# SDU-Gary/PCSS-Unet

Hardware: AMD Instinct MI355X
Metric: frames/sec 7x512x512 U-Net fwd+bwd (train step) (higher is better)
Workload: dtype f32; 1 GPU; configs[1]: batch=8/GPU 7x512x512 fp32 train step (fwd + 0.9*L1 + bwd + RCCL grad all-reduce + clip + AdamW); global_batch=8, in_ch=7, parallelism=dp1

## Files before the change

### include/nsm.h

```cpp
#ifndef NSM_H_
#define NSM_H_

#include <stddef.h>
#include <stdint.h>

#ifdef __cplusplus
extern "C" {
#endif

#define NSM_OK 0
#define NSM_E_ARG 1
#define NSM_E_HIP 2
#define NSM_E_WS 3

#define NSM_F32 0
#define NSM_BF16 1
#define NSM_F16 2

#define NSM_AMAX_WORDS 2048
#define NSM_PACK_FWD 0
#define NSM_PACK_DGRAD 1

int nsm_version(void);
int nsm_get_last_error(char* buf, size_t n);
// ... 84 lines not shown
                      const uint32_t* amax_dy, void* stream);
size_t nsm_wino_wgrad_f16_ws(int B, int H, int W, int cin_p, int cout_p, int tile);
int nsm_conv3x3_wgrad_wino_f16(const void* dM, const void* V, int B, int H, int W, int cin_p,
                               int cout_p, int cin, int cout, int tile, float* dw, float* ws,
                               size_t ws_floats, const uint32_t* amax_dy, const uint32_t* amax_x,
                               void* stream);
int nsm_wino_dual_input_bn_h2(const float* g, int ldg, const float* y, int ldy, int B, int H, int W,
                              int c_p, int tile, const float* scale, const float* shift,
                              float slope, const float* mask, const float* mean, const float* coef,
                              void* Vh, void* dMh, const uint32_t* bound, void* stream);
size_t nsm_wino_wgrad_h2_ws(int B, int H, int W, int cin_p, int cout_p, int tile);
int nsm_conv3x3_wgrad_wino_h2(const void* dMh, const void* Vh, int B, int H, int W, int cin_p,
                              int cout_p, int cin, int cout, int tile, float* dw, float* ws,
                              size_t ws_floats, const uint32_t* amax_dy, const uint32_t* amax_x,
                              void* stream);
int nsm_wino_gemm_h2(const void* V, const void* U, int B, int H, int W, int cin_p, int cout_p,
                     int tile, float* Mb, const uint32_t* amax_v, float beta_v,
                     const uint32_t* amax_u, float beta_u, void* stream);
int nsm_conv1x1_h2_rows(int M, int N, int K, int bnbwd);
int nsm_conv1x1_h2(const void* xh, int M, int cin_p, const void* wh, const float* bias, int cout_p,
                   float* y, int ldy, float* stats, const uint32_t* amax_x,
                   const uint32_t* amax_w, void* stream);
int nsm_conv1x1_dgrad_bnbwd_h2(const void* dy2h, int M, int cop, const void* w2dh, int cip,
                               const float* y1, int ldy1, const float* scale, const float* shift,
                               const float* mean, const float* invstd, const float* mask, int HW,
                               float slope, int mode, float* partial, const float* coef,
                               float* out, int ldo, const uint32_t* amax_dy2,
                               const uint32_t* amax_w, uint32_t* amax_out, uint32_t* amax_k1dz,
                               void* stream);
size_t nsm_conv1x1_wgrad_h2_ws(int M, int cin_p, int cout_p);
int nsm_conv1x1_wgrad_h2(const void* dyh, const void* xh, int M, int cin_p, int cout_p, int cin,
                         int cout, float* dw, float* ws, size_t ws_floats, const uint32_t* amax_dy,
                         const uint32_t* amax_x, void* stream);
int nsm_conv3x3_h2_rows(int M, int N);
int nsm_conv3x3_h2(const void* xh, int B, int H, int W, int cin_p, const void* wh,
                   const float* bias, int cout_p, float* y, int ldy, float* stats,
                   const uint32_t* amax_x, const uint32_t* amax_w, void* stream);
size_t nsm_conv3x3_wgrad_h2_ws(int B, int H, int W, int cin_p, int cout_p);
int nsm_conv3x3_wgrad_h2(const void* dyh, const void* xh, int B, int H, int W, int cin_p,
                         int cout_p, int cin, int cout, float* dw, float* ws, size_t ws_floats,
                         const uint32_t* amax_dy, const uint32_t* amax_x, void* stream);
int nsm_set_f32_split(int mode);
int nsm_wino_output(const float* Mb, int B, int H, int W, int cout_p, int tile, const float* bias,
                    float* y, int ldy, void* stream);
int nsm_wino_output_stats(const float* Mb, int B, int H, int W, int cout_p, int tile,
                          const float* bias, float* y, int ldy, float* partial, int nslot,
                          void* stream);
int nsm_wino_stat_slots(int B, int H, int W, int cout_p, int tile);
int nsm_wino_stat_step(int cout_p, int tile);

size_t nsm_wino_wgrad_ws(int B, int H, int W, int cin_p, int cout_p, int tile);
int nsm_conv3x3_wgrad_wino(const float* dy, int lddy, const float* V, int B, int H, int W,
                           int cin_p, int cout_p, int cin, int cout, int tile, float* dw,
                           float* ws, size_t ws_floats, void* stream);
int nsm_wino_dual_input(const float* dy, int lddy, int B, int H, int W, int c_p, int tile,
                        float* V, float* dM, uint32_t* amax_v, uint32_t* amax_dm, void* stream);
int nsm_wino_dual_input_bn(const float* g, int ldg, const float* y, int ldy, int B, int H, int W,
                           int c_p, int tile, const float* scale, const float* shift, float slope,
                           const float* mask, const float* mean, const float* coef, float* V,
                           float* dM, uint32_t* amax_v, uint32_t* amax_dm, void* stream);
int nsm_conv3x3_wgrad_wino_dm(const float* dM, const float* V, int B, int H, int W, int cin_p,
                              int cout_p, int cin, int cout, int tile, float* dw, float* ws,
                              size_t ws_floats, const uint32_t* amax_dm, const uint32_t* amax_v,
                              void* stream);

size_t nsm_conv_wgrad_ws(int B, int H, int W, int cin_p, int cout_p, int ksize);
int nsm_conv_wgrad(const float* dy, int lddy, const float* x, int ldx, int B, int H, int W,
                   int cin_p, int cout_p, int ksize, const float* pro_scale, const float* pro_shift,
                   const float* pro_mask, float slope, float* ws, size_t ws_floats, int cin, int cout,
                   float* dw, const uint32_t* amax_dy, const uint32_t* amax_x, void* stream);

int nsm_reduce_chunks(int M, int C);
int nsm_reduce_rows(int M, int C);
int nsm_bn_stats(const void* y, int ld, int M, int C, float* partial, int nchunk, int dtype,
                 void* stream);
int nsm_bn_finalize_train(const float* partial, int nchunk, int rows_per_chunk, int M, int C,
                          int c_real,
                          const float* gamma, const float* beta, float* run_mean, float* run_var,
                          int64_t* num_batches, float momentum, float eps, int n_updates,
                          float* mean, float* invstd, float* scale, float* shift, uint32_t* bound,
                          float bound_mul, void* stream);
int nsm_bn_partials_merge(const float* partial, int nchunk, int rows_per_chunk, int M, int C,
                          int group, float* out, void* stream);
int nsm_bn_finalize_eval(const float* run_mean, const float* run_var, const float* gamma,
                         const float* beta, int C, int c_real, float eps, float* mean,
                         float* invstd, float* scale, float* shift, void* stream);
int nsm_bn_act(const void* y, int ldy, int M, int C, const float* scale, const float* shift,
               float slope, const float* mask, int HW, const void* res, int ldres, void* out,
               int ldo, int dtype, uint32_t* amax, void* stream);
int nsm_bn_act_h2(const float* y, int ldy, int M, int C, const float* scale, const float* shift,
                  float slope, const float* mask, int HW, void* out, const uint32_t* bound,
                  void* stream);
int nsm_bn_bwd_reduce(const void* g, int ldg, const void* y, int ldy, int M, int C, int HW,
                      const float* scale, const float* shift, float slope, const float* mask,
                      const float* mean, const float* invstd, float* partial, int nchunk,
                      int dtype, uint32_t* amax_k1dz, void* stream);
int nsm_bn_bwd_finalize(const float* partial, int nchunk, int M, int C, int c_real,
                        const float* gamma, const float* invstd, float* dgamma, float* dbeta,
                        float* dbias_prev, float* coef, const uint32_t* amax_k1dz,
                        uint32_t* bound, void* stream);
int nsm_sum_rows(const float* part, int nrows, int width, int group, float* out, void* stream);
int nsm_bn_bwd_apply(const void* g, int ldg, const void* y, int ldy, int M, int C, int HW,
                     const float* scale, const float* shift, float slope, const float* mask,
                     const float* mean, const float* coef, void* dy, int lddy, int dtype,
                     uint32_t* amax, void* stream);
int nsm_bn_bwd_apply_h2(const float* g, int ldg, const float* y, int ldy, int M, int C, int HW,
                        const float* scale, const float* shift, float slope, const float* mask,
                        const float* mean, const float* coef, void* dy, const uint32_t* bound,
                        void* stream);

int nsm_avgpool2_fwd(const void* x, int B, int H, int W, int C, void* y, int dtype, void* stream);
int nsm_avgpool2_bwd_add(const void* dy, int B, int H, int W, int C, const void* skip, void* dx,
                         int dtype, void* stream);
int nsm_resize_fwd(const void* x, int B, int Hi, int Wi, int C, void* y, int Ho, int Wo, int dtype,
                   void* stream);
int nsm_resize_bwd(const void* dy, int B, int Hi, int Wi, int C, void* dx, int Ho, int Wo,
                   int dtype, void* stream);

int nsm_resize_fwd_act(const void* y2, int B, int Hi, int Wi, int C, void* out, int Ho, int Wo,
                       const float* scale, const float* shift, float slope, const void* res,
                       int dtype, void* stream);
int nsm_up2_resize_fwd_act(const void* y2, int B, int h, int w, int C, void* out, int th, int tw,
                           const float* scale, const float* shift, float slope, const void* res,
                           int dtype, void* stream);
int nsm_bn_act_pool(const void* y, int B, int H, int W, int C, const float* scale,
                    const float* shift, float slope, void* z, void* pooled, int dtype,
                    uint32_t* amax, void* stream);
int nsm_up2_resize_fwd(const void* x, int B, int h, int w, int C, void* y, int th, int tw,
                       int dtype, void* stream);
int nsm_up2_resize_bwd(const void* dy, int B, int h, int w, int C, void* dx, int th, int tw,
                       int dtype, void* stream);
int nsm_bnred_chunks(int kind, int B, int H, int W, int C);
int nsm_avgpool2_bwd_add_bnred(const void* dy, int B, int H, int W, int C, const void* skip,
                               void* dx, int dtype, const void* y2, const float* scale,
                               const float* shift, const float* mean, const float* invstd,
                               float slope, float* partial, uint32_t* amax_k1dz, void* stream);
int nsm_resize_bwd_bnred(const void* dy, int B, int Hi, int Wi, int C, void* dx, int Ho, int Wo,
                         int dtype, const void* y2, const float* scale, const float* shift,
                         const float* mean, const float* invstd, float slope, float* partial,
                         uint32_t* amax_k1dz, void* stream);
int nsm_up2_resize_bwd_bnred(const void* dy, int B, int h, int w, int C, void* dx, int th, int tw,
                             int dtype, const void* y2, const float* scale, const float* shift,
                             const float* mean, const float* invstd, float slope, float* partial,
                             uint32_t* amax_k1dz, void* stream);

int nsm_input_prep(const float* x, int B, int C, int H, int W, void* out, int cp, int dtype,
                   uint32_t* amax, void* stream);
int nsm_input_prep_h2(const float* x, int B, int C, int H, int W, void* out, int cp, uint32_t* amax,
                      void* stream);
int nsm_input_grad(const void* dX, int B, int C, int H, int W, int cp, float* dx, int dtype,
                   void* stream);
int nsm_head_fwd(const void* z, int ldz, int B, int Rh, int Rw, const float* w10,
                 const float* b10, float* out, int dtype, void* stream);
int nsm_head_bwd_blocks(int B, int Rh, int Rw);
int nsm_head_bwd(const float* gout, const float* out, const void* z, int ldz, int B, int Rh,
                 int Rw, const float* w10, void* dz, float* partial, float* dw10, float* db10,
                 int dtype, void* stream);

int nsm_loss_blocks(int64_t n);
int nsm_l1_loss_fwd(const float* o, const float* t, int64_t n, float alpha, float* partial,
                    float* out, void* stream);
int nsm_expdiff_mean(const float* a, const float* b, int64_t n, float alpha, float* partial,
                     float* out, void* stream);
int nsm_l1_loss_bwd(const float* o, const float* t, int64_t n, float alpha, const float* gscale,
                    float* grad, int accumulate, void* stream);
int nsm_detail_blocks(int B, int H, int W);
int nsm_detail_loss_fwd(const float* o, const float* t, int B, int H, int W, float w_hf,
                        float w_pen, float w_sob, const float* base, float* partial, float* out,
                        void* stream);
int nsm_detail_loss_bwd(const float* o, const float* t, int B, int H, int W, float w_hf,
                        float w_pen, float w_sob, const float* mcount, const float* gscale,
                        float* grad, int accumulate, void* stream);
int nsm_ssim_blocks(int B, int H, int W);
int nsm_ssim_fwd(const float* o, const float* t, int B, int H, int W, float data_range, float w,
                 const float* base, float* partial, float* coef, float* out, void* stream);
int nsm_ssim_bwd(const float* o, const float* t, const float* coef, int B, int H, int W, float w,
                 const float* gscale, float* grad, int accumulate, void* stream);
int nsm_temporal_blocks(int B, int C, int H, int W);
int nsm_temporal_pair(const float* cur, const float* prev, const float* mv, const float* depth_cur,
                      const float* depth_prev, const float* normal_cur, const float* normal_prev,
                      int B, int C, int H, int W, float scale_x, float scale_y, float alpha,
                      float depth_tol, float normal_cos, float* psum, int* pcnt, void* stream);
int nsm_temporal_finalize(const float* psum, const int* pcnt, int npairs, int B, int per,
                          int64_t all_count, float* sums, int64_t* counts, float* out, double* acc,
                          void* stream);
int nsm_reproject(const float* prev, const float* mv, int B, int C, int H, int W, float scale_x,
                  float scale_y, float* out, unsigned char* valid, void* stream);
int nsm_taa_resolve(const float* cur, const float* hist, const float* mv, const float* depth_cur,
                    const float* depth_prev, const float* normal_cur, const float* normal_prev,
                    int B, int C, int H, int W, float scale_x, float scale_y, float blend,
                    int clamp, float depth_tol, float normal_cos, float* out,
                    unsigned char* accepted, void* stream);
int nsm_sens_blocks(int64_t n);
int nsm_sens_variants(const float* x, const float* sigma, const int* channels,
                      const float* noises, uint64_t seed, int B, int C, int H, int W, int Cs,
                      int R, float factor, int first, int n, float* out, void* stream);
int nsm_sens_reduce(const float* out, const float* base, int first, int n_slots, int B, int Cs,
                    int R, int64_t n, float* psum, void* stream);
int nsm_sens_finalize(const float* psum, int Cs, int R, int B, int64_t n, const float* sigma,
                      const int* channels, float factor, float* terms, double* acc,
                      float* absolute, float* sgn, float* relative, void* stream);
int nsm_stats_blocks(int64_t hw);
int nsm_stats_partial(const float* x, int B, int C, int64_t HW, double* records, void* stream);
int nsm_stats_merge(const double* records, int B, int C, int per, double* frames, double* state,
                    void* stream);
#define NSM_METRICS_SCALARS 8
int nsm_metrics_blocks(int64_t n);
int nsm_metrics_partial(const float* o, const float* t, int B, int64_t n, float lo, float hi,
                        double* records, void* stream);
int nsm_metrics_merge(const double* records, int B, int per, const float* const* scalars, int K,
                      double* frames, double* log, int64_t log_capacity, double* state,
                      double* acc, void* stream);
int nsm_channel_std(const float* x, int B, int C, int H, int W, float* partial, float* std,
                    void* stream);
int nsm_perturb(const float* x, const float* noise, const float* std, int B, int C, int H,
                int W, float factor, float* out, void* stream);
#define NSM_PERT_MAX 8
int nsm_perturb_variants(const float* x, const float* std, const float* noises, uint64_t seed,
                         const int64_t* seed_dev, int P, int B, int C, int H, int W,
                         float factor, float* out, void* stream);
int nsm_pert_loss_blocks(int64_t n);
int nsm_pert_loss_fwd(const float* o, const float* t, const float* const* pouts, int P, int64_t n,
                      float alpha, float w, const float* vgg, float* partial, float* out,
                      void* stream);
int nsm_pert_loss_bwd(const float* o, const float* t, const float* const* pouts, int P, int64_t n,
                      float alpha, float w, const float* gscale, float* grad, int accumulate,
                      void* stream);

int nsm_sumsq(const float* g, int64_t n, float* partial, float* out, void* stream);
int nsm_clip_coef(const float* sumsq, float inv_world, float max_norm, float* coef, void* stream);
int nsm_adamw_step(float* p, const float* g, float* m, float* v, int64_t n, float lr, float beta1,
                   float beta2, float eps, float weight_decay, int step, const float* gcoef,
                   void* stream);
int nsm_adam_step(float* p, const float* g, float* m, float* v, int64_t n, float lr, float beta1,
                  float beta2, float eps, float weight_decay, int step, const float* gcoef,
                  void* stream);
int nsm_sgd_step(float* p, const float* g, float* buf, int64_t n, float lr, float momentum,
                 float weight_decay, int step, const float* gcoef, void* stream);

#define NSM_SCALER_WORDS 8
// ... 138 lines not shown
```

### pcss-unet_amd/csrc/nsm_elem.hip

```cpp
#include <algorithm>

#include "nsm_common.h"

namespace nsm {

static inline int gcd_i(int a, int b) {
  while (b) {
    int t = a % b;
    a = b;
    b = t;
  }
  return a;
}
struct ColRed {
  int cl, rl, gx, nchunk, rpc;
};
static ColRed colred_plan(int M, int C) {
  ColRed r;
  r.cl = gcd_i(C / 8, 64);
  r.rl = 256 / r.cl;
  r.gx = (C / 8) / r.cl;
  long long want = (M + 63) / 64;
  long long cap = 1024 / r.gx;
  if (cap < 1) cap = 1;
  r.nchunk = (int)(want < cap ? want : cap);
  if (r.nchunk < 1) r.nchunk = 1;
  r.rpc = ceil_div(M, r.nchunk);
  return r;
}

__device__ __forceinline__ void col_tree_reduce(F8* red, int cl, int rl, int tid) {
  for (int s = rl / 2; s > 0; s >>= 1) {
    __syncthreads();
    int tr = tid / cl;
    if (tr < s) red[tid] += red[tid + s * cl];
  }
  __syncthreads();
}

__device__ __forceinline__ F8 ldf8(const float* p) { return ld8(p); }

template <typename T>
__global__ void __launch_bounds__(256) bn_stats_kernel(const T* __restrict__ y, int ld, int M,
                                                       int C, int cl, int rl, int rpc,
                                                       float* __restrict__ partial) {
  __shared__ F8 red[256];
  const int tid = threadIdx.x, tc = tid % cl, tr = tid / cl;
  const int c = (blockIdx.x * cl + tc) * 8;
  const int r0 = blockIdx.y * rpc, r1 = min(M, r0 + rpc);
  F8 s = f8zero();
#pragma unroll 4
  for (int r = r0 + tr; r < r1; r += rl) s += ld8(y + (size_t)r * ld + c);
  red[tid] = s;
  col_tree_reduce(red, cl, rl, tid);
  const float n = (float)max(r1 - r0, 1);
  const F8 sum = red[tc];
  const F8 mean = (1.f / n) * sum;
  __syncthreads();
  F8 s2 = f8zero();
#pragma unroll 4
  for (int r = r0 + tr; r < r1; r += rl) {
    F8 d = ld8(y + (size_t)r * ld + c) - mean;
    s2 += d * d;
  }
  red[tid] = s2;
  col_tree_reduce(red, cl, rl, tid);
  if (tr == 0) {
    float* pr = partial + (size_t)blockIdx.y * 2 * C;
    st8(pr + c, sum);
    st8(pr + C + c, red[tc]);
  }
}

__device__ __forceinline__ double wave_sum_d(double v) {
#pragma unroll
  for (int o = 32; o > 0; o >>= 1) v += __shfl_xor(v, o, 64);
  return v;
}

__device__ __forceinline__ double block_sum_d(double v, double* red) {
  v = wave_sum_d(v);
  __syncthreads();
  if ((threadIdx.x & 63) == 0) red[threadIdx.x >> 6] = v;
  __syncthreads();
  return (red[0] + red[1]) + (red[2] + red[3]);
}

__global__ void __launch_bounds__(256) bn_finalize_train_kernel(
    const float* __restrict__ partial, int nchunk, int rpc, int M, int C, int c_real,
    const float* __restrict__ gamma, const float* __restrict__ beta, float* run_mean,
    float* run_var, int64_t* num_batches, float momentum, float eps, int n_updates, float* mean_o,
    float* invstd_o, float* scale_o, float* shift_o, uint32_t* bound, float bound_mul) {
  __shared__ double red[4];
  const int tid = threadIdx.x;
  const int c = blockIdx.x;
  if (blockIdx.x == 0 && tid == 0 && num_batches) *num_batches += n_updates;
  const size_t st = (size_t)(rpc ? 2 : 3) * C;
  double s0 = 0.0, s1 = 0.0, s2 = 0.0, s3 = 0.0;
  int k = tid;
  for (; k + 768 < nchunk; k += 1024) {
    s0 += partial[k * st + c];
    s1 += partial[(k + 256) * st + c];
    s2 += partial[(k + 512) * st + c];
    s3 += partial[(k + 768) * st + c];
  }
  for (; k < nchunk; k += 256) s0 += partial[k * st + c];
  const double mean = block_sum_d((s0 + s1) + (s2 + s3), red) / M;
  double q0 = 0.0, q1 = 0.0;
  for (k = tid; k < nchunk; k += 512) {
    int n0 = rpc ? min(M, k * rpc + rpc) - k * rpc : (int)partial[k * st + 2 * C + c];
    if (n0 > 0) {
      double d = partial[k * st + c] / n0 - mean;
      q0 += partial[k * st + C + c] + n0 * d * d;
    }
    int k1 = k + 256;
    if (k1 < nchunk) {
      int n1 = rpc ? min(M, k1 * rpc + rpc) - k1 * rpc : (int)partial[k1 * st + 2 * C + c];
      if (n1 > 0) {
        double d = partial[k1 * st + c] / n1 - mean;
        q1 += partial[k1 * st + C + c] + n1 * d * d;
      }
    }
  }
  const double m2 = block_sum_d(q0 + q1, red);
  if (tid != 0) return;
  const float var_b = (float)(m2 / M);
  const float var_u = M > 1 ? (float)(m2 / (M - 1)) : var_b;
  const float mf = (float)mean;
  const float inv = 1.0f / sqrtf(var_b + eps);
  const float sc = gamma[c] * inv;
  mean_o[c] = mf;
  invstd_o[c] = inv;
  scale_o[c] = sc;
  shift_o[c] = beta[c] - mf * sc;
  if (bound) {
    const double b = ((double)fabsf(sc) * sqrt((double)var_b * (double)(M - 1)) +
                      (double)fabsf(beta[c])) * (double)bound_mul * (1.0 + 1e-6);
    atomicMax(bound + (c & (AMAX_LINES - 1)) * AMAX_STRIDE, __float_as_uint((float)b) & 0x7fffffffu);
  }
  if (c < c_real && run_mean) {
    float rm = run_mean[c], rv = run_var[c];
    for (int u = 0; u < n_updates; ++u) {
      rm = momentum * mf + (1.f - momentum) * rm;
      rv = momentum * var_u + (1.f - momentum) * rv;
    }
    run_mean[c] = rm;
    run_var[c] = rv;
  }
}

__global__ void bn_partials_merge_kernel(const float* __restrict__ partial, int nchunk, int rpc,
                                         int M, int C, int G, float* __restrict__ out) {
  const int c = blockIdx.x * blockDim.x + threadIdx.x;
  const int g = blockIdx.y;
  if (c >= C) return;
  const size_t st = (size_t)(rpc ? 2 : 3) * C;
  const int k0 = g * G, k1 = min(nchunk, k0 + G);
  double s = 0.0;
  long long n = 0;
  for (int k = k0; k < k1; ++k) {
    s += partial[(size_t)k * st + c];
    n += rpc ? max(0, min(M, (k + 1) * rpc) - k * rpc) : (long long)partial[(size_t)k * st + 2 * C + c];
  }
  const double mean = n > 0 ? s / (double)n : 0.0;
  double m2 = 0.0;
  for (int k = k0; k < k1; ++k) {
    const int nk = rpc ? min(M, (k + 1) * rpc) - k * rpc : (int)partial[(size_t)k * st + 2 * C + c];
    if (nk <= 0) continue;
    const double d = partial[(size_t)k * st + c] / nk - mean;
    m2 += partial[(size_t)k * st + C + c] + nk * d * d;
  }
  out[(size_t)g * st + c] = (float)s;
  out[(size_t)g * st + C + c] = (float)m2;
  if (!rpc) out[(size_t)g * st + 2 * C + c] = (float)n;
}

__global__ void sum_rows_kernel(const float* __restrict__ part, int nrows, int width, int G,
                                float* __restrict__ out) {
  const int j = blockIdx.x * blockDim.x + threadIdx.x, g = blockIdx.y;
  if (j >= width) return;
  const int k0 = g * G, k1 = min(nrows, k0 + G);
  double s = 0.0, s1 = 0.0;
  int k = k0;
  for (; k + 1 < k1; k += 2) {
    s += part[(size_t)k * width + j];
    s1 += part[(size_t)(k + 1) * width + j];
  }
  if (k < k1) s += part[(size_t)k * width + j];
  out[(size_t)g * width + j] = (float)(s + s1);
}

__global__ void bn_finalize_eval_kernel(const float* __restrict__ rm, const float* __restrict__ rv,
                                        const float* __restrict__ gamma,
                                        const float* __restrict__ beta, int C, int c_real, float eps,
                                        float* mean_o, float* invstd_o, float* scale_o,
                                        float* shift_o) {
  int c = blockIdx.x * blockDim.x + threadIdx.x;
  if (c >= C) return;
  float m = c < c_real ? rm[c] : 0.f;
  float v = c < c_real ? rv[c] : 1.f;
  float inv = 1.0f / sqrtf(v + eps);
  float sc = gamma[c] * inv;
  mean_o[c] = m;
  invstd_o[c] = inv;
  scale_o[c] = sc;
  shift_o[c] = beta[c] - m * sc;
}

__device__ __forceinline__ f32x4 lrelu4(f32x4 v, float slope) {
  return f32x4{lrelu(v.x, slope), lrelu(v.y, slope), lrelu(v.z, slope), lrelu(v.w, slope)};
}
__device__ __forceinline__ F8 lrelu8(F8 v, float slope) {
  return F8{lrelu4(v.a, slope), lrelu4(v.b, slope)};
}

template <typename T>
__global__ void __launch_bounds__(256) bn_act_kernel(const T* __restrict__ y, int ldy, int M,
                                                     int C8, FastDiv fdHW,
                                                     const float* __restrict__ scale,
                                                     const float* __restrict__ shift, float slope,
                                                     const float* __restrict__ mask,
                                                     const T* __restrict__ res, int ldres,
                                                     T* __restrict__ out, int ldo,
                                                     uint32_t* __restrict__ amax) {
  const int ppb = blockDim.x / C8, tp = threadIdx.x / C8;
  const int c = (threadIdx.x - tp * C8) * 8;
  const F8 sc = ldf8(scale + c), sh = ldf8(shift + c);
  const int pstep = gridDim.x * ppb;
  uint32_t am = 0;
  for (int p = blockIdx.x * ppb + tp; p < M; p += pstep) {
    F8 o = lrelu8(ld8(y + (size_t)p * ldy + c) * sc + sh, slope);
    if (mask) o = o * ld8(mask + (size_t)fdiv((uint32_t)p, fdHW) * (C8 * 8) + c);
    if (res) o += ld8(res + (size_t)p * ldres + c);
    st8(out + (size_t)p * ldo + c, o);
    if (amax) {
      amax_fold(am, o.a);
      amax_fold(am, o.b);
    }
  }
  amax_flush(am, amax);
}

__global__ void __launch_bounds__(256) bn_act_h2_kernel(const float* __restrict__ y, int ldy, int M,
                                                        int C8, FastDiv fdHW,
                                                        const float* __restrict__ scale,
                                                        const float* __restrict__ shift,
                                                        float slope,
                                                        const float* __restrict__ mask,
                                                        bf16_t* __restrict__ out, H2Scale hs) {
  const float s = exp2i(h2_exp(hs));
  const int ppb = blockDim.x / C8, tp = threadIdx.x / C8;
  const int c = (threadIdx.x - tp * C8) * 8;
  const F8 sc = ldf8(scale + c), sh = ldf8(shift + c);
  const int pstep = gridDim.x * ppb;
  for (int p = blockIdx.x * ppb + tp; p < M; p += pstep) {
    F8 o = lrelu8(ld8(y + (size_t)p * ldy + c) * sc + sh, slope);
    if (mask) o = o * ld8(mask + (size_t)fdiv((uint32_t)p, fdHW) * (C8 * 8) + c);
    h2_store8(out + (size_t)p * 16 * C8, c, o, s);
  }
}

__device__ __forceinline__ f32x4 lrelu_grad4(f32x4 z, float slope) {
  return f32x4{lrelu_grad(z.x, slope), lrelu_grad(z.y, slope), lrelu_grad(z.z, slope),
               lrelu_grad(z.w, slope)};
}
__device__ __forceinline__ F8 bn_dz8(const F8 g, const F8 v, const F8 sc, const F8 sh,
                                     float slope, const float* mask, int b, int C, int c) {
  const F8 z = v * sc + sh;
  F8 d{g.a * lrelu_grad4(z.a, slope), g.b * lrelu_grad4(z.b, slope)};
  if (mask) d = d * ld8(mask + (size_t)b * C + c);
  return d;
}

template <typename T>
__global__ void __launch_bounds__(256) bn_bwd_reduce_kernel(
    const T* __restrict__ g, int ldg, const T* __restrict__ y, int ldy, int M, int C,
    FastDiv fdHW, const float* __restrict__ scale, const float* __restrict__ shift, float slope,
    const float* __restrict__ mask, const float* __restrict__ mean,
    const float* __restrict__ invstd, int cl, int rl, int rpc, float* __restrict__ partial,
    uint32_t* __restrict__ amax) {
  __shared__ F8 red[256];
  const int tid = threadIdx.x, tc = tid % cl, tr = tid / cl;
  const int c = (blockIdx.x * cl + tc) * 8;
  const int r0 = blockIdx.y * rpc, r1 = min(M, r0 + rpc);
  const F8 sc = ldf8(scale + c), sh = ldf8(shift + c);
  const F8 mu = ldf8(mean + c), is = ldf8(invstd + c);
  F8 s1 = f8zero(), s2 = f8zero();
  uint32_t am = 0;
#pragma unroll 2
  for (int r = r0 + tr; r < r1; r += rl) {
    const F8 v = ld8(y + (size_t)r * ldy + c);
    const F8 gg = ld8(g + (size_t)r * ldg + c);
    const int b = mask ? (int)fdiv((uint32_t)r, fdHW) : 0;
    const F8 dz = bn_dz8(gg, v, sc, sh, slope, mask, b, C, c);
    s1 += dz;
    s2 += dz * ((v - mu) * is);
    if (amax) {
      amax_fold(am, sc.a * dz.a);
      amax_fold(am, sc.b * dz.b);
    }
  }
  amax_flush(am, amax);
  red[tid] = s1;
  col_tree_reduce(red, cl, rl, tid);
  const F8 t1 = red[tc];
  __syncthreads();
  red[tid] = s2;
  col_tree_reduce(red, cl, rl, tid);
  if (tr == 0) {
    float* pr = partial + (size_t)blockIdx.y * 2 * C;
    st8(pr + c, t1);
    st8(pr + C + c, red[tc]);
  }
}

__global__ void __launch_bounds__(256) bn_bwd_finalize_kernel(
    const float* __restrict__ partial, int nchunk, int M, int C, int c_real,
    const float* __restrict__ gamma, const float* __restrict__ invstd, float* dgamma,
    float* dbeta, float* dbias_prev, float* coef, const uint32_t* __restrict__ amax_k1dz,
    uint32_t* __restrict__ bound) {
  __shared__ double red[4];
  const int tid = threadIdx.x;
  const int c = blockIdx.x;
  const float a_k1dz = bound ? __uint_as_float(amax_read(amax_k1dz)) : 0.f;
  const size_t st = (size_t)2 * C;
  double a0 = 0.0, a1 = 0.0, b0 = 0.0, b1 = 0.0;
  int k = tid;
  for (; k + 256 < nchunk; k += 512) {
    a0 += partial[k * st + c];
    b0 += partial[k * st + C + c];
    a1 += partial[(k + 256) * st + c];
    b1 += partial[(k + 256) * st + C + c];
  }
  for (; k < nchunk; k += 256) {
    a0 += partial[k * st + c];
    b0 += partial[k * st + C + c];
  }
  const double S1 = block_sum_d(a0 + a1, red), S2 = block_sum_d(b0 + b1, red);
  if (tid != 0) return;
  const float gm = gamma[c], is = invstd[c];
  const double mdz = S1 / M, mdzx = S2 / M;
  const float k1 = gm * is;
  const float k2 = (float)(-(double)gm * is * is * mdzx);
  const float k3 = (float)(-(double)k1 * mdz);
  coef[c] = k1;
  coef[C + c] = k2;
  coef[2 * C + c] = k3;
  if (bound) {
    const double b = ((double)a_k1dz + fabs((double)k2) * sqrt((double)(M - 1)) / (double)is +
                      fabs((double)k3)) * (1.0 + 1e-6);
    atomicMax(bound + (c & (AMAX_LINES - 1)) * AMAX_STRIDE, __float_as_uint((float)b) & 0x7fffffffu);
  }
  if (c < c_real) {
    if (dgamma) dgamma[c] = (float)S2;
    if (dbeta) dbeta[c] = (float)S1;
    if (dbias_prev) dbias_prev[c] = (float)((double)k1 * S1 + (double)k3 * M);
  }
}

template <typename T>
__global__ void __launch_bounds__(256) bn_bwd_apply_kernel(
    const T* __restrict__ g, int ldg, const T* __restrict__ y, int ldy, int M, int C, int C8,
    FastDiv fdHW, const float* __restrict__ scale, const float* __restrict__ shift, float slope,
    const float* __restrict__ mask, const float* __restrict__ mean,
    const float* __restrict__ coef, T* __restrict__ dy, int lddy, uint32_t* __restrict__ amax) {
  const int ppb = blockDim.x / C8, tp = threadIdx.x / C8;
  const int c = (threadIdx.x - tp * C8) * 8;
  const F8 sc = ldf8(scale + c), sh = ldf8(shift + c), mu = ldf8(mean + c);
  const F8 k1 = ldf8(coef + c), k2 = ldf8(coef + C + c), k3 = ldf8(coef + 2 * C + c);
  const int pstep = gridDim.x * ppb;
  uint32_t am = 0;
  for (int p = blockIdx.x * ppb + tp; p < M; p += pstep) {
    const F8 v = ld8(y + (size_t)p * ldy + c);
    const F8 gg = ld8(g + (size_t)p * ldg + c);
    const int b = mask ? (int)fdiv((uint32_t)p, fdHW) : 0;
    const F8 dz = bn_dz8(gg, v, sc, sh, slope, mask, b, C, c);
    const F8 d = k1 * dz + k2 * (v - mu) + k3;
    st8(dy + (size_t)p * lddy + c, d);
    if (amax) {
      amax_fold(am, d.a);
      amax_fold(am, d.b);
    }
  }
  amax_flush(am, amax);
}

__global__ void __launch_bounds__(256) bn_bwd_apply_h2_kernel(
    const float* __restrict__ g, int ldg, const float* __restrict__ y, int ldy, int M, int C,
    int C8, FastDiv fdHW, const float* __restrict__ scale, const float* __restrict__ shift,
    float slope, const float* __restrict__ mask, const float* __restrict__ mean,
    const float* __restrict__ coef, bf16_t* __restrict__ dy, H2Scale hs) {
  const float s = exp2i(h2_exp(hs));
  const int ppb = blockDim.x / C8, tp = threadIdx.x / C8;
  const int c = (threadIdx.x - tp * C8) * 8;
  const F8 sc = ldf8(scale + c), sh = ldf8(shift + c), mu = ldf8(mean + c);
  const F8 k1 = ldf8(coef + c), k2 = ldf8(coef + C + c), k3 = ldf8(coef + 2 * C + c);
  const int pstep = gridDim.x * ppb;
  for (int p = blockIdx.x * ppb + tp; p < M; p += pstep) {
    const F8 v = ld8(y + (size_t)p * ldy + c);
    const F8 gg = ld8(g + (size_t)p * ldg + c);
    const int b = mask ? (int)fdiv((uint32_t)p, fdHW) : 0;
    const F8 dz = bn_dz8(gg, v, sc, sh, slope, mask, b, C, c);
    h2_store8(dy + (size_t)p * 2 * C, c, k1 * dz + k2 * (v - mu) + k3, s);
  }
}

struct BnRedP {
  const void* y;
  const float* scale;
  const float* shift;
  const float* mean;
  const float* invstd;
  float slope;
  float* partial;
  uint32_t* amax;
};
template <typename T>
__device__ __forceinline__ F8 as_stored8(F8 v);
template <>
__device__ __forceinline__ F8 as_stored8<float>(F8 v) { return v; }
template <>
__device__ __forceinline__ F8 as_stored8<f16_t>(F8 v) {
  const u32x4 w = u32x4{pack_hh(v.a.x, v.a.y), pack_hh(v.a.z, v.a.w), pack_hh(v.b.x, v.b.y),
                        pack_hh(v.b.z, v.b.w)};
  return F8{f32x4{h_lo(w.x), h_hi(w.x), h_lo(w.y), h_hi(w.y)},
            f32x4{h_lo(w.z), h_hi(w.z), h_lo(w.w), h_hi(w.w)}};
}
template <>
__device__ __forceinline__ F8 as_stored8<bf16_t>(F8 v) {
  const u32x4 w = u32x4{pack_bf2(v.a.x, v.a.y), pack_bf2(v.a.z, v.a.w), pack_bf2(v.b.x, v.b.y),
                        pack_bf2(v.b.z, v.b.w)};
  return F8{f32x4{bf_lo(w.x), bf_hi(w.x), bf_lo(w.y), bf_hi(w.y)},
            f32x4{bf_lo(w.z), bf_hi(w.z), bf_lo(w.w), bf_hi(w.w)}};
}
struct BnRedAcc {
  F8 sc, sh, mu, is, s1, s2;
  uint32_t am;
  __device__ void init(const BnRedP& r, int c) {
    sc = ldf8(r.scale + c);
    sh = ldf8(r.shift + c);
    mu = ldf8(r.mean + c);
    is = ldf8(r.invstd + c);
    s1 = f8zero();
    s2 = f8zero();
    am = 0;
  }
  template <typename T>
  __device__ void add(const BnRedP& r, F8 g, size_t p, int C, int c) {
    const F8 v = ld8((const T*)r.y + p * C + c);
    const F8 dz = bn_dz8(g, v, sc, sh, r.slope, nullptr, 0, C, c);
    s1 += dz;
    s2 += dz * ((v - mu) * is);
    if (r.amax) {
      amax_fold(am, sc.a * dz.a);
      amax_fold(am, sc.b * dz.b);
    }
  }
  __device__ void write(const BnRedP& r, int C8) {
    __shared__ F8 red[256];
    const int tid = threadIdx.x, rl = 256 / C8, tc = tid % C8, C = C8 * 8;
    red[tid] = s1;
    col_tree_reduce(red, C8, rl, tid);
    const F8 t1 = red[tc];
    __syncthreads();
    red[tid] = s2;
    col_tree_reduce(red, C8, rl, tid);
    if (tid < C8) {
      float* pr = r.partial + (size_t)blockIdx.x * 2 * C;
      st8(pr + tc * 8, t1);
      st8(pr + C + tc * 8, red[tc]);
    }
    amax_flush(am, r.amax);
  }
  __device__ void write_slice(const BnRedP& r, int G, int c0, int C, int row) {
    __shared__ F8 red[256];
    const int tid = threadIdx.x, rl = 256 / G, tc = tid % G;
    red[tid] = s1;
    col_tree_reduce(red, G, rl, tid);
    const F8 t1 = red[tc];
    __syncthreads();
    red[tid] = s2;
    col_tree_reduce(red, G, rl, tid);
    if (tid < G) {
      float* pr = r.partial + (size_t)row * 2 * C + c0;
      st8(pr + tc * 8, t1);
      st8(pr + C + tc * 8, red[tc]);
    }
    amax_flush(am, r.amax);
  }
};

template <typename T>
__global__ void __launch_bounds__(256) avgpool2_fwd_kernel(const T* __restrict__ x, int B, int H,
                                                           int W, int C8, FastDiv fdC8,
                                                           FastDiv fdWo, FastDiv fdHo,
                                                           T* __restrict__ y) {
  const int Ho = H / 2, Wo = W / 2, C = C8 * 8;
  const uint32_t total = (uint32_t)B * Ho * Wo * C8;
  for (uint32_t i = blockIdx.x * 256u + threadIdx.x; i < total; i += gridDim.x * 256u) {
    const uint32_t p = fdiv(i, fdC8);
    const int c = (int)(i - p * (uint32_t)C8) * 8;
    const uint32_t t = fdiv(p, fdWo);
    const int ox = (int)(p - t * Wo);
    const uint32_t b = fdiv(t, fdHo);
    const int oy = (int)(t - b * Ho);
    const T* base = x + (((size_t)b * H + 2 * oy) * W + 2 * ox) * C + c;
    const size_t rs = (size_t)W * C;
    F8 s = ld8(base);
    s += ld8(base + C);
    s += ld8(base + rs);
    s += ld8(base + rs + C);
    st8(y + (size_t)p * C + c, 0.25f * s);
  }
}

template <typename T>
__global__ void __launch_bounds__(256) bn_act_pool_kernel(const T* __restrict__ y, int B, int H,
                                                          int W, int C8, FastDiv fdC8,
                                                          FastDiv fdWc, FastDiv fdHc,
                                                          const float* __restrict__ scale,
                                                          const float* __restrict__ shift,
                                                          float slope, T* __restrict__ z,
                                                          T* __restrict__ pooled,
                                                          uint32_t* __restrict__ amax) {
  const int Hc = (H + 1) / 2, Wc = (W + 1) / 2, Ho = H / 2, Wo = W / 2, C = C8 * 8;
  uint32_t am = 0;
  const uint32_t total = (uint32_t)B * Hc * Wc * C8;
  for (uint32_t i = blockIdx.x * 256u + threadIdx.x; i < total; i += gridDim.x * 256u) {
    const uint32_t p = fdiv(i, fdC8);
    const int c = (int)(i - p * (uint32_t)C8) * 8;
    const uint32_t t = fdiv(p, fdWc);
    const int cx = (int)(p - t * Wc);
// ... 783 lines not shown
template <bool COMP>
static void dispatch_sep_bwd(const SepPlan& pl, int B, size_t lds, hipStream_t s, const void* dy,
                             int h, int w, int C, void* dx, int th, int tw, float s1h, float s1w,
                             float s2h, float s2w, const BnRedP* rp, int dtype) {
  const dim3 g((unsigned)(B * ((h + pl.R - 1) / pl.R)), (unsigned)(C >> (pl.lcb8 + 3)));
  const BnRedP r = rp ? *rp : BnRedP{};
#define NSM_SEP(T, RED, R)                                                                      \
  launch_sep_bwd<T, RED, COMP, R>(g, lds, s, dy, h, w, C, pl.lcb8, dx, th, tw, s1h, s1w, s2h, s2w, r)
#define NSM_SEP_R(T, RED) \
  (pl.R == 4 ? NSM_SEP(T, RED, 4) : pl.R == 2 ? NSM_SEP(T, RED, 2) : NSM_SEP(T, RED, 1))
  if (dtype == NSM_BF16) {
    if (rp) NSM_SEP_R(bf16_t, true); else NSM_SEP_R(bf16_t, false);
  }
  else if (dtype == NSM_F16) {
    if (rp) NSM_SEP_R(f16_t, true); else NSM_SEP_R(f16_t, false);
  } else {
    if (rp) NSM_SEP_R(float, true); else NSM_SEP_R(float, false);
  }
#undef NSM_SEP_R
#undef NSM_SEP
}
static int sep_resize_mode() { static const int v = (int)env_int("NSM_RESIZE_SEP", 1); return v; }
static bool sep_resize() { return sep_resize_mode() != 0; }
static bool sep_for(int dtype) { return dtype == NSM_F32 ? sep_resize() : sep_resize_mode() == 2; }

template <typename T, bool H2 = false>
__global__ void __launch_bounds__(256) input_prep_kernel(const float* __restrict__ x, int B, int C,
                                                         int H, int W, T* __restrict__ out, int cp,
                                                         uint32_t npix, FastDiv fdRw, FastDiv fdRh,
                                                         uint32_t* __restrict__ amax) {
  const int Rh = H / 2, Rw = W / 2;
  const size_t plane = (size_t)H * W;
  float hs = 0.f;
  if constexpr (H2) hs = exp2i(h2_exp(H2Scale{amax, 1.f}));
  uint32_t am = 0;
  for (uint32_t p = blockIdx.x * 256u + threadIdx.x; p < npix; p += gridDim.x * 256u) {
    const uint32_t t = fdiv(p, fdRw);
    const int rx = (int)(p - t * (uint32_t)Rw);
    const uint32_t b = fdiv(t, fdRh);
    const int ry = (int)(t - b * (uint32_t)Rh);
    const float* src = x + (size_t)b * C * plane + (size_t)(2 * ry) * W + 2 * rx;
    for (int g = 0; g < cp / 8; ++g) {
      f32x2 r[4];
#pragma unroll
      for (int q = 0; q < 4; ++q) {
        const int c = 2 * g + (q >> 1);
        r[q] = c < C ? *(const f32x2*)(src + (size_t)c * plane + (q & 1) * W) : f32x2{0.f, 0.f};
      }
      const F8 v{f32x4{r[0].x, r[0].y, r[1].x, r[1].y}, f32x4{r[2].x, r[2].y, r[3].x, r[3].y}};
      if constexpr (H2) {
        h2_store8((bf16_t*)out + (size_t)p * 2 * cp, 8 * g, v, hs);
      } else {
        st8(out + (size_t)p * cp + 8 * g, v);
        if (amax) {
          amax_fold(am, v.a);
          amax_fold(am, v.b);
        }
      }
    }
  }
  if constexpr (!H2) amax_flush(am, amax);
}

template <typename T>
__global__ void input_grad_kernel(const T* __restrict__ dX, int B, int C, int H, int W, int cp,
                                  float* __restrict__ dx) {
  const int Rh = H / 2, Rw = W / 2;
  long long total = (long long)B * C * Rh * Rw;
  long long i = (long long)blockIdx.x * blockDim.x + threadIdx.x;
  for (; i < total; i += (long long)gridDim.x * blockDim.x) {
    int rx = (int)(i % Rw);
    long long t = i / Rw;
    int ry = (int)(t % Rh);
    t /= Rh;
    int c = (int)(t % C);
    int b = (int)(t / C);
    f32x4 v = ld4(dX + (((size_t)b * Rh + ry) * Rw + rx) * cp + 4 * c);
    float* o = dx + (((size_t)b * C + c) * H + 2 * ry) * W + 2 * rx;
    *(f32x2*)o = f32x2{v.x, v.y};
    *(f32x2*)(o + W) = f32x2{v.z, v.w};
  }
}

template <typename T>
__global__ void head_fwd_kernel(const T* __restrict__ z, int ldz, int B, int Rh, int Rw,
                                const float* __restrict__ w10, const float* __restrict__ b10,
                                float* __restrict__ out) {
  __shared__ float w[68];
  if (threadIdx.x < 64) w[threadIdx.x] = w10[threadIdx.x];
  if (threadIdx.x < 4) w[64 + threadIdx.x] = b10[threadIdx.x];
  __syncthreads();
  long long npix = (long long)B * Rh * Rw;
  for (long long p = (long long)blockIdx.x * blockDim.x + threadIdx.x; p < npix;
       p += (long long)gridDim.x * blockDim.x) {
    float zz[16];
    const T* zr = z + (size_t)p * ldz;
#pragma unroll
    for (int q = 0; q < 4; ++q) {
      f32x4 v = ld4(zr + 4 * q);
      zz[4 * q] = v.x;
      zz[4 * q + 1] = v.y;
      zz[4 * q + 2] = v.z;
      zz[4 * q + 3] = v.w;
    }
    int rx = (int)(p % Rw);
    long long t = p / Rw;
    int ry = (int)(t % Rh);
    int b = (int)(t / Rh);
#pragma unroll
    for (int j = 0; j < 4; ++j) {
      float acc = 0.f;
#pragma unroll
      for (int c = 0; c < 16; ++c) acc += w[j * 16 + c] * zz[c];
      acc += w[64 + j];
      float s = 1.f / (1.f + expf(-acc));
      int di = j >> 1, dj = j & 1;
      out[((size_t)b * 2 * Rh + 2 * ry + di) * (2 * Rw) + 2 * rx + dj] = s;
    }
  }
}

__device__ __forceinline__ float wave_sum(float v) {
#pragma unroll
  for (int o = 32; o > 0; o >>= 1) v += __shfl_xor(v, o, 64);
  return v;
}

template <typename T>
__global__ void __launch_bounds__(256) head_bwd_kernel(
    const float* __restrict__ gout, const float* __restrict__ out, const T* __restrict__ z,
    int ldz, int B, int Rh, int Rw, const float* __restrict__ w10, T* __restrict__ dz,
    float* __restrict__ partial) {
  __shared__ float w[64];
  __shared__ float red[4][68];
  if (threadIdx.x < 64) w[threadIdx.x] = w10[threadIdx.x];
  __syncthreads();
  float accw[68];
#pragma unroll
  for (int k = 0; k < 68; ++k) accw[k] = 0.f;
  long long npix = (long long)B * Rh * Rw;
  for (long long p = (long long)blockIdx.x * blockDim.x + threadIdx.x; p < npix;
       p += (long long)gridDim.x * blockDim.x) {
    int rx = (int)(p % Rw);
    long long t = p / Rw;
    int ry = (int)(t % Rh);
    int b = (int)(t / Rh);
    float d[4];
#pragma unroll
    for (int di = 0; di < 2; ++di) {
      size_t o = ((size_t)b * 2 * Rh + 2 * ry + di) * (2 * Rw) + 2 * rx;
      const f32x2 ov = *(const f32x2*)(out + o), gv = *(const f32x2*)(gout + o);
      d[2 * di] = gv.x * (1.f - ov.x) * ov.x;
      d[2 * di + 1] = gv.y * (1.f - ov.y) * ov.y;
    }
    const T* zr = z + (size_t)p * ldz;
    T* dzr = dz + (size_t)p * ldz;
#pragma unroll
    for (int q = 0; q < 4; ++q) {
      f32x4 v = ld4(zr + 4 * q);
      float zv[4] = {v.x, v.y, v.z, v.w};
      f32x4 g;
      float gv[4];
#pragma unroll
      for (int e = 0; e < 4; ++e) {
        int c = 4 * q + e;
        gv[e] = d[0] * w[c] + d[1] * w[16 + c] + d[2] * w[32 + c] + d[3] * w[48 + c];
#pragma unroll
        for (int j = 0; j < 4; ++j) accw[j * 16 + c] += d[j] * zv[e];
      }
      g.x = gv[0];
      g.y = gv[1];
      g.z = gv[2];
      g.w = gv[3];
      st4(dzr + 4 * q, g);
    }
    for (int c = 16; c < ldz; c += 4) st4(dzr + c, f32x4{0.f, 0.f, 0.f, 0.f});
#pragma unroll
    for (int j = 0; j < 4; ++j) accw[64 + j] += d[j];
  }
  const int lane = threadIdx.x & 63, wv = threadIdx.x >> 6;
#pragma unroll
  for (int o = 32; o >= 1; o >>= 1) {
    const bool up = (lane & o) != 0;
#pragma unroll
    for (int i = 0; i < o; ++i) {
      const float lo = accw[i], hi = accw[i + o];
      accw[i] = (up ? hi : lo) + __shfl_xor(up ? lo : hi, o, 64);
    }
  }
  red[wv][lane] = accw[0];
#pragma unroll
  for (int k = 64; k < 68; ++k) {
    float s = wave_sum(accw[k]);
    if (lane == 0) red[wv][k] = s;
  }
  __syncthreads();
  if (threadIdx.x < 68) {
    float s = red[0][threadIdx.x] + red[1][threadIdx.x] + red[2][threadIdx.x] + red[3][threadIdx.x];
    partial[(size_t)blockIdx.x * 68 + threadIdx.x] = s;
  }
}

__global__ void __launch_bounds__(256) head_reduce_kernel(const float* __restrict__ partial,
                                                          int nblk, float* dw10, float* db10) {
  __shared__ double sh[256];
  const int j = blockIdx.x;
  double s = 0.0;
  for (int b = threadIdx.x; b < nblk; b += 256) s += partial[(size_t)b * 68 + j];
  sh[threadIdx.x] = s;
  __syncthreads();
  for (int o = 128; o > 0; o >>= 1) {
    if ((int)threadIdx.x < o) sh[threadIdx.x] += sh[threadIdx.x + o];
    __syncthreads();
  }
  if (threadIdx.x == 0) {
    if (j < 64)
      dw10[j] = (float)sh[0];
    else
      db10[j - 64] = (float)sh[0];
  }
}

__device__ __forceinline__ float block_sum256(float v, float* sh) {
  v = wave_sum(v);
  const int lane = threadIdx.x & 63, wv = threadIdx.x >> 6;
  __syncthreads();
  if (lane == 0) sh[wv] = v;
  __syncthreads();
  float r = 0.f;
  if (threadIdx.x == 0) {
    for (int k = 0; k < (int)(blockDim.x >> 6); ++k) r += sh[k];
  }
  return r;
}

__global__ void __launch_bounds__(256) l1_partial_kernel(const float* __restrict__ o,
                                                         const float* __restrict__ t, int64_t n,
                                                         float* __restrict__ partial) {
  __shared__ float sh[4];
  float s = 0.f;
  for (int64_t i = (int64_t)blockIdx.x * blockDim.x + threadIdx.x; i < n;
       i += (int64_t)gridDim.x * blockDim.x)
    s += fabsf(o[i] - t[i]);
  float r = block_sum256(s, sh);
  if (threadIdx.x == 0) partial[blockIdx.x] = r;
}

__global__ void __launch_bounds__(256) expdiff_partial_kernel(const float* __restrict__ a,
                                                              const float* __restrict__ b,
                                                              int64_t n, float alpha,
                                                              float* __restrict__ partial) {
  __shared__ float sh[4];
  float s = 0.f;
  for (int64_t i = (int64_t)blockIdx.x * blockDim.x + threadIdx.x; i < n;
       i += (int64_t)gridDim.x * blockDim.x)
    s += expf(alpha * fabsf(a[i] - b[i])) - 1.f;
  float r = block_sum256(s, sh);
  if (threadIdx.x == 0) partial[blockIdx.x] = r;
}

__global__ void finalize_mean_kernel(const float* __restrict__ partial, int nblk, double scale,
                                     float* out) {
  __shared__ double sh[64];
  double s = 0.0;
  for (int b = threadIdx.x; b < nblk; b += 64) s += partial[b];
  sh[threadIdx.x] = s;
  __syncthreads();
  if (threadIdx.x == 0) {
    double tot = 0.0;
    for (int k = 0; k < 64; ++k) tot += sh[k];
    out[0] = (float)(tot * scale);
  }
}

__global__ void l1_bwd_kernel(const float* __restrict__ o, const float* __restrict__ t, int64_t n,
                              float alpha, const float* __restrict__ gscale, float* grad,
                              int accumulate) {
  const float gs = gscale ? gscale[0] : 1.f;
  const float mag = (alpha * gs) / (float)n;
  for (int64_t i = (int64_t)blockIdx.x * blockDim.x + threadIdx.x; i < n;
       i += (int64_t)gridDim.x * blockDim.x) {
    float d = o[i] - t[i];
// ... 125 lines not shown
                           float* __restrict__ buf, int64_t n, float lr, float momentum, float wd,
                           int first, const float* __restrict__ gcoef) {
#pragma clang fp contract(off)
  const float gc = gcoef ? gcoef[0] : 1.f;
  for (int64_t i = (int64_t)blockIdx.x * blockDim.x + threadIdx.x; i < n;
       i += (int64_t)gridDim.x * blockDim.x) {
    float pi = p[i];
    float gi = g[i] * gc;
    gi = gi + wd * pi;
    if (MOMENTUM) {
      if (!first) gi = buf[i] * momentum + gi;
      buf[i] = gi;
    }
    p[i] = pi - lr * gi;
  }
}

static inline int xcd_grid(long long work) {
  long long g = (work + 255) / 256;
  g = g > 2048 ? 2048 : g;
  return (int)((g + 7) / 8 * 8);
}

static inline int grid_for(long long work, int per_block = 256, int cap = 8192) {
  long long g = (work + per_block - 1) / per_block;
  if (g < 1) g = 1;
  if (g > cap) g = cap;
  return (int)g;
}

}

using namespace nsm;

extern "C" int nsm_reduce_chunks(int M, int C) {
  if (M <= 0 || C <= 0 || C % 8) return 0;
  return colred_plan(M, C).nchunk;
}

#define NSM_T(T, p) ((T*)(p))
#define NSM_CT(T, p) ((const T*)(p))

extern "C" int nsm_bn_stats(const void* y, int ld, int M, int C, float* partial, int nchunk,
                            int dtype, void* stream) {
  NSM_CHECK_ARG(y && partial && M > 0 && C % 8 == 0 && ld % 8 == 0, "bn_stats: bad args");
  ColRed r = colred_plan(M, C);
  NSM_CHECK_ARG(nchunk == r.nchunk, "bn_stats: nchunk %d != %d", nchunk, r.nchunk);
  dim3 g(r.gx, r.nchunk);
  if (dtype == NSM_BF16)
    hipLaunchKernelGGL(bn_stats_kernel<bf16_t>, g, dim3(256), 0, as_stream(stream),
                       NSM_CT(bf16_t, y), ld, M, C, r.cl, r.rl, r.rpc, partial);
  else if (dtype == NSM_F16)
    hipLaunchKernelGGL(bn_stats_kernel<f16_t>, g, dim3(256), 0, as_stream(stream),
                       NSM_CT(f16_t, y), ld, M, C, r.cl, r.rl, r.rpc, partial);
  else
    hipLaunchKernelGGL(bn_stats_kernel<float>, g, dim3(256), 0, as_stream(stream),
                       NSM_CT(float, y), ld, M, C, r.cl, r.rl, r.rpc, partial);
  NSM_LAUNCH_CHECK("bn_stats");
  return 0;
}

extern "C" int nsm_reduce_rows(int M, int C) {
  if (M <= 0 || C <= 0 || C % 8) return 0;
  return colred_plan(M, C).rpc;
}

extern "C" int nsm_bn_finalize_train(const float* partial, int nchunk, int rows_per_chunk, int M,
                                     int C, int c_real, const float* gamma, const float* beta,
                                     float* run_mean, float* run_var, int64_t* num_batches,
                                     float momentum, float eps, int n_updates, float* mean,
                                     float* invstd, float* scale, float* shift, uint32_t* bound,
                                     float bound_mul, void* stream) {
  NSM_CHECK_ARG(partial && gamma && beta && mean && invstd && scale && shift, "bn_finalize: null");
  NSM_CHECK_ARG(M > 1, "bn_finalize: Expected more than 1 value per channel when training");
  NSM_CHECK_ARG(nchunk >= 1 && (rows_per_chunk == 0 ||
                                (rows_per_chunk >= 1 && (long long)nchunk * rows_per_chunk >= M)),
                "bn_finalize: chunks do not cover M");
  hipLaunchKernelGGL(bn_finalize_train_kernel, dim3(C), dim3(256), 0,
                     as_stream(stream), partial, nchunk, rows_per_chunk, M, C, c_real, gamma, beta,
                     run_mean,
                     run_var, num_batches, momentum, eps, n_updates, mean, invstd, scale, shift,
                     bound, bound_mul);
  NSM_LAUNCH_CHECK("bn_finalize_train");
  return 0;
}

extern "C" int nsm_bn_partials_merge(const float* partial, int nchunk, int rows_per_chunk, int M,
                                     int C, int group, float* out, void* stream) {
  NSM_CHECK_ARG(partial && out && nchunk >= 1 && group >= 1 && rows_per_chunk >= 0,
                "bn_partials_merge: bad args");
  dim3 grid(ceil_div(C, 256), ceil_div(nchunk, group));
  hipLaunchKernelGGL(bn_partials_merge_kernel, grid, dim3(256), 0, as_stream(stream), partial,
                     nchunk, rows_per_chunk, M, C, group, out);
  NSM_LAUNCH_CHECK("bn_partials_merge");
  return 0;
}

extern "C" int nsm_sum_rows(const float* part, int nrows, int width, int group, float* out,
                            void* stream) {
  NSM_CHECK_ARG(part && out && nrows >= 1 && width >= 1 && group >= 1, "sum_rows: bad args");
  dim3 grid(ceil_div(width, 256), ceil_div(nrows, group));
  hipLaunchKernelGGL(sum_rows_kernel, grid, dim3(256), 0, as_stream(stream), part, nrows, width,
                     group, out);
  NSM_LAUNCH_CHECK("sum_rows");
  return 0;
}

extern "C" int nsm_bn_finalize_eval(const float* run_mean, const float* run_var,
                                    const float* gamma, const float* beta, int C, int c_real,
                                    float eps, float* mean, float* invstd, float* scale,
                                    float* shift, void* stream) {
  NSM_CHECK_ARG(run_mean && run_var && gamma && beta && scale && shift, "bn_finalize_eval: null");
  hipLaunchKernelGGL(bn_finalize_eval_kernel, dim3(ceil_div(C, 256)), dim3(256), 0,
                     as_stream(stream), run_mean, run_var, gamma, beta, C, c_real, eps, mean, invstd,
                     scale, shift);
  NSM_LAUNCH_CHECK("bn_finalize_eval");
  return 0;
}

static void pix_launch(long long M, int C8, dim3& grid, dim3& block) {
  const int tpb = (256 / C8) * C8;
  const long long ppb = tpb / C8;
  long long g = (M + ppb - 1) / ppb;
  g = g < 1 ? 1 : (g > 2048 ? 2048 : g);
  grid = dim3((unsigned)g);
  block = dim3((unsigned)tpb);
}

extern "C" int nsm_bn_act(const void* y, int ldy, int M, int C, const float* scale,
                          const float* shift, float slope, const float* mask, int HW,
                          const void* res, int ldres, void* out, int ldo, int dtype,
                          uint32_t* amax, void* stream) {
  NSM_CHECK_ARG(y && scale && shift && out && C % 8 == 0 && C <= 2048 && ldy % 8 == 0 &&
                    ldo % 8 == 0 && (!res || ldres % 8 == 0) && (!mask || HW > 0),
                "bn_act: bad args");
  NSM_CHECK_ARG(M >= 0 && M < (1 << 30), "bn_act: too large");
  if (M == 0) return 0;
  dim3 g, b;
  pix_launch(M, C / 8, g, b);
  const FastDiv fh = make_fastdiv(mask ? HW : 1);
  if (dtype == NSM_BF16)
    hipLaunchKernelGGL(bn_act_kernel<bf16_t>, g, b, 0, as_stream(stream), NSM_CT(bf16_t, y), ldy,
                       M, C / 8, fh, scale, shift, slope, mask, NSM_CT(bf16_t, res), ldres,
                       NSM_T(bf16_t, out), ldo, amax);
  else if (dtype == NSM_F16)
    hipLaunchKernelGGL(bn_act_kernel<f16_t>, g, b, 0, as_stream(stream), NSM_CT(f16_t, y), ldy,
                       M, C / 8, fh, scale, shift, slope, mask, NSM_CT(f16_t, res), ldres,
                       NSM_T(f16_t, out), ldo, amax);
  else
    hipLaunchKernelGGL(bn_act_kernel<float>, g, b, 0, as_stream(stream), NSM_CT(float, y), ldy, M,
                       C / 8, fh, scale, shift, slope, mask, NSM_CT(float, res), ldres,
                       NSM_T(float, out), ldo, amax);
  NSM_LAUNCH_CHECK("bn_act");
  return 0;
}

extern "C" int nsm_bn_act_h2(const float* y, int ldy, int M, int C, const float* scale,
                             const float* shift, float slope, const float* mask, int HW, void* out,
                             const uint32_t* bound, void* stream) {
  NSM_CHECK_ARG(y && scale && shift && out && bound && C % 8 == 0 && C <= 2048 && ldy % 8 == 0 &&
                    (!mask || HW > 0) && ((uintptr_t)out % 16) == 0,
                "bn_act_h2: bad args");
  NSM_CHECK_ARG(M >= 0 && M < (1 << 30), "bn_act_h2: too large");
  if (M == 0) return 0;
  dim3 g, b;
  pix_launch(M, C / 8, g, b);
  hipLaunchKernelGGL(bn_act_h2_kernel, g, b, 0, as_stream(stream), y, ldy, M, C / 8,
                     make_fastdiv(mask ? HW : 1), scale, shift, slope, mask, (bf16_t*)out,
                     H2Scale{bound, 1.f});
  NSM_LAUNCH_CHECK("bn_act_h2");
  return 0;
}

extern "C" int nsm_bn_bwd_reduce(const void* g, int ldg, const void* y, int ldy, int M, int C,
                                 int HW, const float* scale, const float* shift, float slope,
                                 const float* mask, const float* mean, const float* invstd,
                                 float* partial, int nchunk, int dtype, uint32_t* amax_k1dz,
                                 void* stream) {
  NSM_CHECK_ARG(g && y && scale && shift && mean && invstd && partial && C % 8 == 0 &&
                    ldg % 8 == 0 && ldy % 8 == 0, "bn_bwd_reduce: bad args");
  ColRed r = colred_plan(M, C);
  NSM_CHECK_ARG(nchunk == r.nchunk, "bn_bwd_reduce: nchunk mismatch");
  dim3 gr(r.gx, r.nchunk);
  if (dtype == NSM_BF16)
    hipLaunchKernelGGL(bn_bwd_reduce_kernel<bf16_t>, gr, dim3(256), 0, as_stream(stream),
                       NSM_CT(bf16_t, g), ldg, NSM_CT(bf16_t, y), ldy, M, C, make_fastdiv(HW),
                       scale, shift, slope, mask, mean, invstd, r.cl, r.rl, r.rpc, partial,
                       amax_k1dz);
  else if (dtype == NSM_F16)
    hipLaunchKernelGGL(bn_bwd_reduce_kernel<f16_t>, gr, dim3(256), 0, as_stream(stream),
                       NSM_CT(f16_t, g), ldg, NSM_CT(f16_t, y), ldy, M, C, make_fastdiv(HW),
                       scale, shift, slope, mask, mean, invstd, r.cl, r.rl, r.rpc, partial,
                       amax_k1dz);
  else
    hipLaunchKernelGGL(bn_bwd_reduce_kernel<float>, gr, dim3(256), 0, as_stream(stream),
                       NSM_CT(float, g), ldg, NSM_CT(float, y), ldy, M, C, make_fastdiv(HW), scale,
                       shift, slope, mask, mean, invstd, r.cl, r.rl, r.rpc, partial, amax_k1dz);
  NSM_LAUNCH_CHECK("bn_bwd_reduce");
  return 0;
}

extern "C" int nsm_bn_bwd_finalize(const float* partial, int nchunk, int M, int C, int c_real,
                                   const float* gamma, const float* invstd, float* dgamma,
                                   float* dbeta, float* dbias_prev, float* coef,
                                   const uint32_t* amax_k1dz, uint32_t* bound, void* stream) {
  NSM_CHECK_ARG(partial && gamma && invstd && coef, "bn_bwd_finalize: bad args");
  NSM_CHECK_ARG(!bound || amax_k1dz, "bn_bwd_finalize: a bound needs the max|k1 dz| slot");
  NSM_CHECK_ARG(M > 1 || !bound, "bn_bwd_finalize: M");
  hipLaunchKernelGGL(bn_bwd_finalize_kernel, dim3(C), dim3(256), 0,
                     as_stream(stream), partial, nchunk, M, C, c_real, gamma, invstd, dgamma, dbeta,
                     dbias_prev, coef, amax_k1dz, bound);
  NSM_LAUNCH_CHECK("bn_bwd_finalize");
  return 0;
}

extern "C" int nsm_bn_bwd_apply(const void* g, int ldg, const void* y, int ldy, int M, int C,
                                int HW, const float* scale, const float* shift, float slope,
                                const float* mask, const float* mean, const float* coef, void* dy,
                                int lddy, int dtype, uint32_t* amax, void* stream) {
  NSM_CHECK_ARG(g && y && scale && shift && mean && coef && dy && C % 8 == 0 && C <= 2048 &&
                    ldg % 8 == 0 && ldy % 8 == 0 && lddy % 8 == 0 && (!mask || HW > 0),
                "bn_bwd_apply: bad args");
  NSM_CHECK_ARG(M >= 0 && M < (1 << 30), "bn_bwd_apply: too large");
  if (M == 0) return 0;
  dim3 gr, b;
  pix_launch(M, C / 8, gr, b);
  const FastDiv fh = make_fastdiv(mask ? HW : 1);
  if (dtype == NSM_BF16)
    hipLaunchKernelGGL(bn_bwd_apply_kernel<bf16_t>, gr, b, 0, as_stream(stream),
                       NSM_CT(bf16_t, g), ldg, NSM_CT(bf16_t, y), ldy, M, C, C / 8, fh, scale,
                       shift, slope, mask, mean, coef, NSM_T(bf16_t, dy), lddy, amax);
  else if (dtype == NSM_F16)
    hipLaunchKernelGGL(bn_bwd_apply_kernel<f16_t>, gr, b, 0, as_stream(stream),
                       NSM_CT(f16_t, g), ldg, NSM_CT(f16_t, y), ldy, M, C, C / 8, fh, scale,
                       shift, slope, mask, mean, coef, NSM_T(f16_t, dy), lddy, amax);
  else
    hipLaunchKernelGGL(bn_bwd_apply_kernel<float>, gr, b, 0, as_stream(stream),
                       NSM_CT(float, g), ldg, NSM_CT(float, y), ldy, M, C, C / 8, fh, scale,
                       shift, slope, mask, mean, coef, NSM_T(float, dy), lddy, amax);
  NSM_LAUNCH_CHECK("bn_bwd_apply");
  return 0;
}

extern "C" int nsm_bn_bwd_apply_h2(const float* g, int ldg, const float* y, int ldy, int M, int C,
                                   int HW, const float* scale, const float* shift, float slope,
                                   const float* mask, const float* mean, const float* coef,
                                   void* dy, const uint32_t* bound, void* stream) {
  NSM_CHECK_ARG(g && y && scale && shift && mean && coef && dy && bound && C % 8 == 0 &&
                    C <= 2048 && ldg % 8 == 0 && ldy % 8 == 0 && (!mask || HW > 0) &&
                    ((uintptr_t)dy % 16) == 0,
                "bn_bwd_apply_h2: bad args");
  NSM_CHECK_ARG(M >= 0 && M < (1 << 30), "bn_bwd_apply_h2: too large");
  if (M == 0) return 0;
  dim3 gr, b;
  pix_launch(M, C / 8, gr, b);
  hipLaunchKernelGGL(bn_bwd_apply_h2_kernel, gr, b, 0, as_stream(stream), g, ldg, y, ldy, M, C,
                     C / 8, make_fastdiv(mask ? HW : 1), scale, shift, slope, mask, mean, coef,
                     (bf16_t*)dy, H2Scale{bound, 1.f});
  NSM_LAUNCH_CHECK("bn_bwd_apply_h2");
  return 0;
}

extern "C" int nsm_bn_act_pool(const void* y, int B, int H, int W, int C, const float* scale,
                               const float* shift, float slope, void* z, void* pooled, int dtype,
                               uint32_t* amax, void* stream) {
  NSM_CHECK_ARG(y && z && pooled && scale && shift && C % 8 == 0 && H >= 2 && W >= 2,
                "bn_act_pool: bad args");
  const long long work = (long long)B * ((H + 1) / 2) * ((W + 1) / 2) * (C / 8);
  NSM_CHECK_ARG(work < (1ll << 31), "bn_act_pool: too large");
  dim3 g(grid_for(work));
  const FastDiv f8 = make_fastdiv(C / 8), fw = make_fastdiv((W + 1) / 2),
                fh = make_fastdiv((H + 1) / 2);
  if (dtype == NSM_BF16)
    hipLaunchKernelGGL(bn_act_pool_kernel<bf16_t>, g, dim3(256), 0, as_stream(stream),
                       NSM_CT(bf16_t, y), B, H, W, C / 8, f8, fw, fh, scale, shift, slope,
                       NSM_T(bf16_t, z), NSM_T(bf16_t, pooled), amax);
  else if (dtype == NSM_F16)
    hipLaunchKernelGGL(bn_act_pool_kernel<f16_t>, g, dim3(256), 0, as_stream(stream),
                       NSM_CT(f16_t, y), B, H, W, C / 8, f8, fw, fh, scale, shift, slope,
                       NSM_T(f16_t, z), NSM_T(f16_t, pooled), amax);
  else
    hipLaunchKernelGGL(bn_act_pool_kernel<float>, g, dim3(256), 0, as_stream(stream),
                       NSM_CT(float, y), B, H, W, C / 8, f8, fw, fh, scale, shift, slope,
                       NSM_T(float, z), NSM_T(float, pooled), amax);
  NSM_LAUNCH_CHECK("bn_act_pool");
  return 0;
}

extern "C" int nsm_avgpool2_fwd(const void* x, int B, int H, int W, int C, void* y, int dtype,
                                void* stream) {
  NSM_CHECK_ARG(x && y && C % 8 == 0 && H >= 2 && W >= 2, "avgpool2_fwd: bad args");
  long long work = (long long)B * (H / 2) * (W / 2) * (C / 8);
  NSM_CHECK_ARG(work < (1ll << 31), "avgpool2_fwd: too large");
  dim3 g(grid_for(work));
  const FastDiv f8 = make_fastdiv(C / 8), fw = make_fastdiv(W / 2), fh = make_fastdiv(H / 2);
// ... 338 lines not shown
                                          void* stream) {
  NSM_BNRED_CHECK("avgpool2_bwd_add_bnred");
  return avgpool2_bwd_add(dy, B, H, W, C, skip, dx, dtype, &rp, stream);
}
extern "C" int nsm_resize_bwd_bnred(const void* dy, int B, int Hi, int Wi, int C, void* dx, int Ho,
                                    int Wo, int dtype, NSM_BNRED_ARGS, void* stream) {
  NSM_BNRED_CHECK("resize_bwd_bnred");
  return resize_bwd(dy, B, Hi, Wi, C, dx, Ho, Wo, dtype, &rp, stream);
}
extern "C" int nsm_up2_resize_bwd_bnred(const void* dy, int B, int h, int w, int C, void* dx,
                                        int th, int tw, int dtype, NSM_BNRED_ARGS, void* stream) {
  NSM_BNRED_CHECK("up2_resize_bwd_bnred");
  return up2_resize_bwd(dy, B, h, w, C, dx, th, tw, dtype, &rp, stream);
}
#undef NSM_BNRED_ARGS
#undef NSM_BNRED_CHECK
#undef NSM_DT

extern "C" int nsm_input_prep(const float* x, int B, int C, int H, int W, void* out, int cp,
                              int dtype, uint32_t* amax, void* stream) {
  NSM_CHECK_ARG(x && out && H % 2 == 0 && W % 2 == 0 && cp >= 4 * C && cp % 8 == 0,
                "input_prep: bad args");
  NSM_CHECK_ARG(((uintptr_t)x % 8) == 0, "input_prep: x must be 8-byte aligned");
  const long long npix = (long long)B * (H / 2) * (W / 2);
  NSM_CHECK_ARG(npix < (1ll << 31), "input_prep: too large");
  dim3 g(grid_for(npix, 256, 2048));
  const FastDiv fw = make_fastdiv(W / 2), fh = make_fastdiv(H / 2);
  if (dtype == NSM_BF16)
    hipLaunchKernelGGL(input_prep_kernel<bf16_t>, g, dim3(256), 0, as_stream(stream), x, B, C, H, W,
                       NSM_T(bf16_t, out), cp, (uint32_t)npix, fw, fh, nullptr);
  else if (dtype == NSM_F16)
    hipLaunchKernelGGL(input_prep_kernel<f16_t>, g, dim3(256), 0, as_stream(stream), x, B, C, H, W,
                       NSM_T(f16_t, out), cp, (uint32_t)npix, fw, fh, nullptr);
  else
    hipLaunchKernelGGL(input_prep_kernel<float>, g, dim3(256), 0, as_stream(stream), x, B, C, H, W,
                       NSM_T(float, out), cp, (uint32_t)npix, fw, fh, amax);
  NSM_LAUNCH_CHECK("input_prep");
  return 0;
}

extern "C" int nsm_input_prep_h2(const float* x, int B, int C, int H, int W, void* out, int cp,
                                 uint32_t* amax, void* stream) {
  NSM_CHECK_ARG(x && out && amax && H % 2 == 0 && W % 2 == 0 && cp >= 4 * C && cp % 8 == 0,
                "input_prep_h2: bad args");
  NSM_CHECK_ARG(((uintptr_t)x % 8) == 0 && ((uintptr_t)out % 16) == 0, "input_prep_h2: alignment");
  const long long npix = (long long)B * (H / 2) * (W / 2);
  NSM_CHECK_ARG(npix < (1ll << 31), "input_prep_h2: too large");
  const int rc = nsm_absmax(x, (int64_t)B * C * H * W, amax, stream);
  if (rc) return rc;
  dim3 g(grid_for(npix, 256, 2048));
  hipLaunchKernelGGL((input_prep_kernel<bf16_t, true>), g, dim3(256), 0, as_stream(stream), x, B, C,
                     H, W, (bf16_t*)out, cp, (uint32_t)npix, make_fastdiv(W / 2),
                     make_fastdiv(H / 2), amax);
  NSM_LAUNCH_CHECK("input_prep_h2");
  return 0;
}

extern "C" int nsm_input_grad(const void* dX, int B, int C, int H, int W, int cp, float* dx,
                              int dtype, void* stream) {
  NSM_CHECK_ARG(dX && dx && H % 2 == 0 && W % 2 == 0 && cp >= 4 * C && cp % 4 == 0,
                "input_grad: bad args");
  long long work = (long long)B * C * (H / 2) * (W / 2);
  dim3 g(grid_for(work));
  if (dtype == NSM_BF16)
    hipLaunchKernelGGL(input_grad_kernel<bf16_t>, g, dim3(256), 0, as_stream(stream),
                       NSM_CT(bf16_t, dX), B, C, H, W, cp, dx);
  else if (dtype == NSM_F16)
    hipLaunchKernelGGL(input_grad_kernel<f16_t>, g, dim3(256), 0, as_stream(stream),
                       NSM_CT(f16_t, dX), B, C, H, W, cp, dx);
  else
    hipLaunchKernelGGL(input_grad_kernel<float>, g, dim3(256), 0, as_stream(stream),
                       NSM_CT(float, dX), B, C, H, W, cp, dx);
  NSM_LAUNCH_CHECK("input_grad");
  return 0;
}

extern "C" int nsm_head_fwd(const void* z, int ldz, int B, int Rh, int Rw, const float* w10,
                            const float* b10, float* out, int dtype, void* stream) {
  NSM_CHECK_ARG(z && w10 && b10 && out && ldz >= 16 && ldz % 4 == 0, "head_fwd: bad args");
  long long npix = (long long)B * Rh * Rw;
  dim3 g(grid_for(npix));
  if (dtype == NSM_BF16)
    hipLaunchKernelGGL(head_fwd_kernel<bf16_t>, g, dim3(256), 0, as_stream(stream),
                       NSM_CT(bf16_t, z), ldz, B, Rh, Rw, w10, b10, out);
  else if (dtype == NSM_F16)
    hipLaunchKernelGGL(head_fwd_kernel<f16_t>, g, dim3(256), 0, as_stream(stream),
                       NSM_CT(f16_t, z), ldz, B, Rh, Rw, w10, b10, out);
  else
    hipLaunchKernelGGL(head_fwd_kernel<float>, g, dim3(256), 0, as_stream(stream),
                       NSM_CT(float, z), ldz, B, Rh, Rw, w10, b10, out);
  NSM_LAUNCH_CHECK("head_fwd");
  return 0;
}

extern "C" int nsm_head_bwd_blocks(int B, int Rh, int Rw) {
  return grid_for((long long)B * Rh * Rw, 256, 1024);
}

extern "C" int nsm_head_bwd(const float* gout, const float* out, const void* z, int ldz, int B,
                            int Rh, int Rw, const float* w10, void* dz, float* partial, float* dw10,
                            float* db10, int dtype, void* stream) {
  NSM_CHECK_ARG(gout && out && z && w10 && dz && partial && dw10 && db10 && ldz % 4 == 0,
                "head_bwd: bad args");
  int nblk = nsm_head_bwd_blocks(B, Rh, Rw);
  hipStream_t s = as_stream(stream);
  if (dtype == NSM_BF16)
    hipLaunchKernelGGL(head_bwd_kernel<bf16_t>, dim3(nblk), dim3(256), 0, s, gout, out,
                       NSM_CT(bf16_t, z), ldz, B, Rh, Rw, w10, NSM_T(bf16_t, dz), partial);
  else if (dtype == NSM_F16)
    hipLaunchKernelGGL(head_bwd_kernel<f16_t>, dim3(nblk), dim3(256), 0, s, gout, out,
                       NSM_CT(f16_t, z), ldz, B, Rh, Rw, w10, NSM_T(f16_t, dz), partial);
  else
    hipLaunchKernelGGL(head_bwd_kernel<float>, dim3(nblk), dim3(256), 0, s, gout, out,
                       NSM_CT(float, z), ldz, B, Rh, Rw, w10, NSM_T(float, dz), partial);
  NSM_LAUNCH_CHECK("head_bwd");
  hipLaunchKernelGGL(head_reduce_kernel, dim3(68), dim3(256), 0, s, partial, nblk, dw10, db10);
  NSM_LAUNCH_CHECK("head_reduce");
  return 0;
}

extern "C" int nsm_loss_blocks(int64_t n) { return grid_for(n, 1024, 1024); }

extern "C" int nsm_l1_loss_fwd(const float* o, const float* t, int64_t n, float alpha,
                               float* partial, float* out, void* stream) {
  NSM_CHECK_ARG(o && t && partial && out && n > 0, "l1_loss_fwd: bad args");
  int nb = nsm_loss_blocks(n);
  hipStream_t s = as_stream(stream);
  hipLaunchKernelGGL(l1_partial_kernel, dim3(nb), dim3(256), 0, s, o, t, n, partial);
  hipLaunchKernelGGL(finalize_mean_kernel, dim3(1), dim3(64), 0, s, partial, nb,
                     (double)alpha / (double)n, out);
  NSM_LAUNCH_CHECK("l1_loss_fwd");
  return 0;
}

extern "C" int nsm_expdiff_mean(const float* a, const float* b, int64_t n, float alpha,
                                float* partial, float* out, void* stream) {
  NSM_CHECK_ARG(a && b && partial && out && n > 0, "expdiff_mean: bad args");
  int nb = nsm_loss_blocks(n);
  hipStream_t s = as_stream(stream);
  hipLaunchKernelGGL(expdiff_partial_kernel, dim3(nb), dim3(256), 0, s, a, b, n, alpha, partial);
  hipLaunchKernelGGL(finalize_mean_kernel, dim3(1), dim3(64), 0, s, partial, nb, 1.0 / (double)n,
                     out);
  NSM_LAUNCH_CHECK("expdiff_mean");
  return 0;
}

extern "C" int nsm_l1_loss_bwd(const float* o, const float* t, int64_t n, float alpha,
                               const float* gscale, float* grad, int accumulate, void* stream) {
  NSM_CHECK_ARG(o && t && grad && n > 0, "l1_loss_bwd: bad args");
  hipLaunchKernelGGL(l1_bwd_kernel, dim3(grid_for(n)), dim3(256), 0, as_stream(stream), o, t, n,
                     alpha, gscale, grad, accumulate);
  NSM_LAUNCH_CHECK("l1_loss_bwd");
  return 0;
}

extern "C" int nsm_channel_std(const float* x, int B, int C, int H, int W, float* partial,
                               float* std_o, void* stream) {
  (void)partial;
  NSM_CHECK_ARG(x && std_o && B * H * W > 0, "channel_std: bad args");
  hipLaunchKernelGGL(channel_std_kernel, dim3(C), dim3(1024), 0, as_stream(stream), x, B, C, H * W,
                     std_o);
  NSM_LAUNCH_CHECK("channel_std");
  return 0;
}

extern "C" int nsm_perturb(const float* x, const float* noise, const float* stdv, int B, int C,
                           int H, int W, float factor, float* out, void* stream) {
  NSM_CHECK_ARG(x && noise && stdv && out, "perturb: bad args");
  long long total = (long long)B * C * H * W;
  hipLaunchKernelGGL(perturb_kernel, dim3(grid_for(total)), dim3(256), 0, as_stream(stream), x,
                     noise, stdv, C, H * W, total, factor, out);
  NSM_LAUNCH_CHECK("perturb");
  return 0;
}

extern "C" int nsm_normalize_frames(float* x, int B, int C, int64_t HW, const float* mean,
                                    const float* stdv, float eps, void* stream) {
  NSM_CHECK_ARG(x && mean && stdv && B > 0 && C > 0 && HW > 0, "normalize_frames: bad args");
  long long total = (long long)B * C * HW;
  hipLaunchKernelGGL(normalize_frames_kernel, dim3(grid_for(total)), dim3(256), 0,
                     as_stream(stream), x, C, (long long)HW, total, mean, stdv, eps);
  NSM_LAUNCH_CHECK("normalize_frames");
  return 0;
}

extern "C" int nsm_sumsq(const float* g, int64_t n, float* partial, float* out, void* stream) {
  NSM_CHECK_ARG(g && partial && out && n > 0, "sumsq: bad args");
  int nb = nsm_loss_blocks(n);
  hipStream_t s = as_stream(stream);
  hipLaunchKernelGGL(sumsq_partial_kernel, dim3(nb), dim3(256), 0, s, g, n, partial);
  hipLaunchKernelGGL(finalize_mean_kernel, dim3(1), dim3(64), 0, s, partial, nb, 1.0, out);
  NSM_LAUNCH_CHECK("sumsq");
  return 0;
}

extern "C" int nsm_clip_coef(const float* sumsq, float inv_world, float max_norm, float* coef,
                             void* stream) {
// ... 262 lines not shown
```

### pcss-unet_amd/nsm_amd/_lib.py

```python
import ctypes
import os

import torch

_HERE = os.path.dirname(os.path.abspath(__file__))
LIB_PATH = os.environ.get("NSM_LIB", os.path.join(_HERE, "libnsm.so"))

P = ctypes.c_void_p
I = ctypes.c_int
L = ctypes.c_int64
F = ctypes.c_float
Z = ctypes.c_size_t
D = ctypes.c_double
U64 = ctypes.c_uint64

_SIGS = {
    "nsm_version": (I, []),
    "nsm_get_last_error": (I, [ctypes.c_char_p, Z]),
    "nsm_pack_conv_weight": (I, [P, I, I, I, I, I, I, P, P]),
    "nsm_pad_vec": (I, [P, I, I, P, P]),
    "nsm_conv_fwd": (I, [P, I, I, I, I, I, P, P, I, I, P, I, P, P, P, F, P]),
    "nsm_conv_stat_rows": (I, [I, I, I, I]),
    "nsm_conv_fwd_stats": (I, [P, I, I, I, I, I, P, P, I, I, P, I, P, P, P, F, P, P, P, P]),
    "nsm_wino_ws": (Z, [I, I, I, I, I, I]),
    "nsm_wino_weight": (I, [P, I, I, I, I, I, I, P, P]),
    "nsm_conv3x3_wino": (I, [P, I, I, I, I, I, P, P, I, I, I, P, I, P, Z, P]),
    "nsm_wino_input": (I, [P, I, I, I, I, I, I, I, P, P]),
    "nsm_wino_gemm": (I, [P, P, I, I, I, I, I, I, P, P]),
    "nsm_wino_gemm_s": (I, [P, P, I, I, I, I, I, I, P, P, P, P]),
    "nsm_absmax": (I, [P, L, P, P]),
    "nsm_zero_u32": (I, [P, L, P]),
    "nsm_absmax_bf16": (I, [P, L, P, P]),
    "nsm_pmc_calib": (I, [I, P, P, L, P]),
    "nsm_to_h2": (I, [P, L, I, P, F, P, P]),
    "nsm_wino_gemm_h2": (I, [P, P, I, I, I, I, I, I, P, P, F, P, F, P]),
    "nsm_wino_beta": (F, [I, I]),
    "nsm_wino_input_h2": (I, [P, I, I, I, I, I, I, I, I, P, P, P]),
    "nsm_wino_dual_input_h2": (I, [P, I, I, I, I, I, I, P, P, P, P]),
    "nsm_wino_dual_input_bn_h2": (I, [P, I, P, I, I, I, I, I, I, P, P, F, P, P, P, P, P, P, P]),
    "nsm_wino_input_f16": (I, [P, I, I, I, I, I, I, P, P, P]),
    "nsm_wino_input_f16_resize": (I, [P, I, I, I, I, I, I, I, I, P, P, P]),
    "nsm_wino_gemm_f16": (I, [P, P, I, I, I, I, I, I, P, P, F, P, F, P]),
    "nsm_wino_output_bf16": (I, [P, I, I, I, I, I, P, P, I, P, I, P]),
    "nsm_wino_gemm_f16m": (I, [P, P, I, I, I, I, I, I, P, P, P, F, P, F, P]),
    "nsm_wino_output_bf16m": (I, [P, P, I, I, I, I, I, I, P, F, P, F, P, P, I, P, I, P]),
    "nsm_wino_output_bf16m_act": (I, [P, P, I, I, I, I, I, I, P, F, P, F, P, P, I, P, P, F, P]),
    "nsm_wino_dout_f16": (I, [P, I, I, I, I, I, I, P, P, P]),
    "nsm_wino_dual_f16": (I, [P, I, I, I, I, I, I, P, P, P, P]),
    "nsm_wino_dual_bn_f16": (I, [P, I, P, I, I, I, I, I, I, P, P, F, P, P, P, P, P, P, P]),
    "nsm_wino_wgrad_f16_ws": (Z, [I, I, I, I, I, I]),
    "nsm_conv3x3_wgrad_wino_f16": (I, [P, P, I, I, I, I, I, I, I, I, P, P, Z, P, P, P]),
    "nsm_wino_wgrad_h2_ws": (Z, [I, I, I, I, I, I]),
    "nsm_conv3x3_wgrad_wino_h2": (I, [P, P, I, I, I, I, I, I, I, I, P, P, Z, P, P, P]),
    "nsm_set_f32_split": (I, [I]),
    "nsm_wino_output": (I, [P, I, I, I, I, I, P, P, I, P]),
    "nsm_wino_wgrad_ws": (Z, [I, I, I, I, I, I]),
    "nsm_conv3x3_wgrad_wino": (I, [P, I, P, I, I, I, I, I, I, I, I, P, P, Z, P]),
    "nsm_conv_wgrad_ws": (Z, [I, I, I, I, I, I]),
    "nsm_conv_wgrad": (I, [P, I, P, I, I, I, I, I, I, I, P, P, P, F, P, Z, I, I, P, P, P, P]),
    "nsm_reduce_chunks": (I, [I, I]),
    "nsm_reduce_rows": (I, [I, I]),
    "nsm_bn_stats": (I, [P, I, I, I, P, I, I, P]),
    "nsm_bn_finalize_train": (I, [P, I, I, I, I, I, P, P, P, P, P, F, F, I, P, P, P, P, P, F, P]),
    "nsm_bn_act_h2": (I, [P, I, I, I, P, P, F, P, I, P, P, P]),
    "nsm_conv1x1_h2_rows": (I, [I, I, I, I]),
    "nsm_conv1x1_h2": (I, [P, I, I, P, P, I, P, I, P, P, P, P]),
    "nsm_conv1x1_dgrad_bnbwd_h2": (I, [P, I, I, P, I, P, I, P, P, P, P, P, I, F, I, P, P, P, I, P,
                                       P, P, P, P]),
    "nsm_conv3x3_h2_rows": (I, [I, I]),
    "nsm_conv3x3_h2": (I, [P, I, I, I, I, P, P, I, P, I, P, P, P, P]),
    "nsm_conv3x3_wgrad_h2_ws": (Z, [I, I, I, I, I]),
    "nsm_conv3x3_wgrad_h2": (I, [P, P, I, I, I, I, I, I, I, P, P, Z, P, P, P]),
    "nsm_input_prep_h2": (I, [P, I, I, I, I, P, I, P, P]),
    "nsm_conv1x1_wgrad_h2_ws": (Z, [I, I, I]),
    "nsm_conv1x1_wgrad_h2": (I, [P, P, I, I, I, I, I, P, P, Z, P, P, P]),
    "nsm_bn_partials_merge": (I, [P, I, I, I, I, I, P, P]),
    "nsm_bn_finalize_eval": (I, [P, P, P, P, I, I, F, P, P, P, P, P]),
    "nsm_bn_act": (I, [P, I, I, I, P, P, F, P, I, P, I, P, I, I, P, P]),
    "nsm_bn_bwd_reduce": (I, [P, I, P, I, I, I, I, P, P, F, P, P, P, P, I, I, P, P]),
    "nsm_bn_bwd_finalize": (I, [P, I, I, I, I, P, P, P, P, P, P, P, P, P]),
    "nsm_bn_bwd_apply_h2": (I, [P, I, P, I, I, I, I, P, P, F, P, P, P, P, P, P]),
    "nsm_bn_bwd_apply": (I, [P, I, P, I, I, I, I, P, P, F, P, P, P, P, I, I, P, P]),
    "nsm_sum_rows": (I, [P, I, I, I, P, P]),
    "nsm_resize_fwd_act": (I, [P, I, I, I, I, P, I, I, P, P, F, P, I, P]),
    "nsm_up2_resize_fwd_act": (I, [P, I, I, I, I, P, I, I, P, P, F, P, I, P]),
    "nsm_bn_act_pool": (I, [P, I, I, I, I, P, P, F, P, P, I, P, P]),
    "nsm_wino_dual_input": (I, [P, I, I, I, I, I, I, P, P, P, P, P]),
    "nsm_wino_dual_input_bn": (I, [P, I, P, I, I, I, I, I, I, P, P, F, P, P, P, P, P, P, P, P]),
    "nsm_conv3x3_wgrad_wino_dm": (I, [P, P, I, I, I, I, I, I, I, I, P, P, Z, P, P, P]),
    "nsm_conv_fwd_act": (I, [P, I, I, I, I, I, P, P, I, I, P, I, P, P, F, P, I, I, P]),
    "nsm_wino_output_act": (I, [P, I, I, I, I, I, P, P, I, P, P, F, P, I, P]),
    "nsm_bnred_chunks": (I, [I, I, I, I, I]),
    "nsm_avgpool2_bwd_add_bnred": (I, [P, I, I, I, I, P, P, I, P, P, P, P, P, F, P, P, P]),
    "nsm_resize_bwd_bnred": (I, [P, I, I, I, I, P, I, I, I, P, P, P, P, P, F, P, P, P]),
    "nsm_up2_resize_bwd_bnred": (I, [P, I, I, I, I, P, I, I, I, P, P, P, P, P, F, P, P, P]),
    "nsm_wino_input_resize": (I, [P, I, I, I, I, I, I, I, I, I, P, P, P]),
    "nsm_wino_output_stats": (I, [P, I, I, I, I, I, P, P, I, P, I, P]),
    "nsm_wino_stat_slots": (I, [I, I, I, I, I]),
    "nsm_wino_stat_step": (I, [I, I]),
    "nsm_conv1x1_bnbwd_chunks": (I, [I, I, I, I, I, I]),
    "nsm_conv1x1_dgrad_bnbwd": (I, [P, I, I, I, I, I, P, I, P, I, P, P, P, P, P, F, I, P, P, P, I,
                                    I, P, P, P, P]),
    "nsm_avgpool2_fwd": (I, [P, I, I, I, I, P, I, P]),
    "nsm_avgpool2_bwd_add": (I, [P, I, I, I, I, P, P, I, P]),
    "nsm_resize_fwd": (I, [P, I, I, I, I, P, I, I, I, P]),
    "nsm_resize_bwd": (I, [P, I, I, I, I, P, I, I, I, P]),
    "nsm_up2_resize_fwd": (I, [P, I, I, I, I, P, I, I, I, P]),
    "nsm_up2_resize_bwd": (I, [P, I, I, I, I, P, I, I, I, P]),
    "nsm_input_prep": (I, [P, I, I, I, I, P, I, I, P, P]),
    "nsm_input_grad": (I, [P, I, I, I, I, I, P, I, P]),
    "nsm_head_fwd": (I, [P, I, I, I, I, P, P, P, I, P]),
    "nsm_head_bwd_blocks": (I, [I, I, I]),
    "nsm_head_bwd": (I, [P, P, P, I, I, I, I, P, P, P, P, P, I, P]),
    "nsm_loss_blocks": (I, [L]),
    "nsm_l1_loss_fwd": (I, [P, P, L, F, P, P, P]),
    "nsm_expdiff_mean": (I, [P, P, L, F, P, P, P]),
    "nsm_l1_loss_bwd": (I, [P, P, L, F, P, P, I, P]),
    "nsm_detail_blocks": (I, [I, I, I]),
    "nsm_detail_loss_fwd": (I, [P, P, I, I, I, F, F, F, P, P, P, P]),
    "nsm_detail_loss_bwd": (I, [P, P, I, I, I, F, F, F, P, P, P, I, P]),
    "nsm_ssim_blocks": (I, [I, I, I]),
    "nsm_ssim_fwd": (I, [P, P, I, I, I, F, F, P, P, P, P, P]),
    "nsm_ssim_bwd": (I, [P, P, P, I, I, I, F, P, P, I, P]),
    "nsm_temporal_blocks": (I, [I, I, I, I]),
    "nsm_temporal_pair": (I, [P, P, P, P, P, P, P, I, I, I, I, F, F, F, F, F, P, P, P]),
    "nsm_temporal_finalize": (I, [P, P, I, I, I, L, P, P, P, P, P]),
    "nsm_reproject": (I, [P, P, I, I, I, I, F, F, P, P, P]),
    "nsm_taa_resolve": (I, [P, P, P, P, P, P, P, I, I, I, I, F, F, F, I, F, F, P, P, P]),
    "nsm_sens_blocks": (I, [L]),
    "nsm_sens_variants": (I, [P, P, P, P, U64, I, I, I, I, I, I, F, I, I, P, P]),
    "nsm_sens_reduce": (I, [P, P, I, I, I, I, I, L, P, P]),
    "nsm_sens_finalize": (I, [P, I, I, I, L, P, P, F, P, P, P, P, P, P]),
    "nsm_stats_blocks": (I, [L]),
    "nsm_stats_partial": (I, [P, I, I, L, P, P]),
    "nsm_stats_merge": (I, [P, I, I, I, P, P, P]),
    "nsm_metrics_blocks": (I, [L]),
    "nsm_metrics_partial": (I, [P, P, I, L, F, F, P, P]),
    "nsm_metrics_merge": (I, [P, I, I, P, I, P, P, L, P, P, P]),
    "nsm_channel_std": (I, [P, I, I, I, I, P, P, P]),
    "nsm_perturb": (I, [P, P, P, I, I, I, I, F, P, P]),
    "nsm_perturb_variants": (I, [P, P, P, U64, P, I, I, I, I, I, F, P, P]),
    "nsm_pert_loss_blocks": (I, [L]),
    "nsm_pert_loss_fwd": (I, [P, P, P, I, L, F, F, P, P, P, P]),
    "nsm_pert_loss_bwd": (I, [P, P, P, I, L, F, F, P, P, I, P]),
    "nsm_sumsq": (I, [P, L, P, P, P]),
    "nsm_clip_coef": (I, [P, F, F, P, P]),
    "nsm_adamw_step": (I, [P, P, P, P, L, F, F, F, F, F, I, P, P]),
    "nsm_adam_step": (I, [P, P, P, P, L, F, F, F, F, F, I, P, P]),
    "nsm_sgd_step": (I, [P, P, P, L, F, F, F, I, P, P]),
    "nsm_vgg_prep": (I, [P, P, I, I, I, F, F, P, P]),
    "nsm_npy_info": (I, [ctypes.c_char_p, P, I, P, P, P]),
    "nsm_loader_create": (P, [ctypes.c_char_p, ctypes.c_char_p, I, I, I, I, I]),
    "nsm_loader_batches": (L, [P]),
    "nsm_loader_frame_dims": (I, [P, P, P, P]),
    "nsm_loader_next": (I, [P, P, P, P]),
    "nsm_loader_destroy": (None, [P]),
    "nsm_normalize_frames": (I, [P, I, I, L, P, P, F, P]),
    "nsm_frame_blocks": (I, [I, I, I]),
    "nsm_frame_prep": (I, [P, I, I, I, I, I, I, P, P, F, I, P, P, P, P]),
    "nsm_frame_finish": (I, [P, I, I, I, I, I, I, P, P, P, P, P]),
    "nsm_pack_conv_weight_bf16": (I, [P, I, I, I, I, I, I, P, P]),
    "nsm_conv_fwd_bf16": (I, [P, I, I, I, I, I, P, P, I, I, P, I, P, P, P, F, P, P]),
    "nsm_conv_wgrad_bf16_ws": (Z, [I, I, I, I, I, I]),
    "nsm_conv_stat_rows_bf16": (I, [I, I, I, I]),
    "nsm_conv_wgrad_bf16": (I, [P, I, P, I, I, I, I, I, I, I, P, P, P, F, P, Z, I, I, P, P]),
    "nsm_pack_conv_weight_f16": (I, [P, I, I, I, I, I, I, P, P]),
    "nsm_conv_fwd_f16": (I, [P, I, I, I, I, I, P, P, I, I, P, I, P, P, P, F, P, P]),
    "nsm_conv_wgrad_f16": (I, [P, I, P, I, I, I, I, I, I, I, P, P, P, F, P, Z, I, I, P, P]),
    "nsm_maxpool2_fwd": (I, [P, I, I, I, I, P, P]),
    "nsm_vgg_tap_relu_bwd": (I, [P, P, P, L, F, P, I, I, P]),
    "nsm_maxpool2_bwd": (I, [P, P, P, I, I, I, I, F, P, P, P]),
    "nsm_vgg_prep_bwd": (I, [P, P, I, I, I, F, F, P, I, P]),
    "nsm_tail_chunk": (L, []),
    "nsm_tail_plan": (I, [P, I, P, P, P, P, I]),
    "nsm_tail_ws_bytes": (Z, [I, I]),
    "nsm_grad_tail": (I, [P, I, P, P, P, P, P, I, F, F, F, P, U64, P, Z, P, P, P, P, P]),
    "nsm_grad_tail_scaled": (I, [P, I, P, P, P, P, P, I, F, P, F, P, U64, P, Z, P, P, P, P, F, F,
                                 I, I, P]),
    "nsm_scaler_set": (I, [P, F, I, P]),
    "nsm_adamw_tail": (I, [P, P, P, P, P, P, P, I, P, P, P, D, D, D, D, D, P]),
    "nsm_adam_tail": (I, [P, P, P, P, P, P, P, I, P, P, P, D, D, D, D, D, P]),
    "nsm_sgd_tail": (I, [P, P, P, P, P, P, I, P, P, P, D, D, D, P]),
    "nsm_hyper_bytes": (Z, []),
    "nsm_hyper_set": (I, [P, D, F, P]),
    "nsm_grad_tail_dev": (I, [P, I, P, P, P, P, P, I, F, F, P, P, U64, P, Z, P, P, P, P, P]),
    "nsm_grad_tail_scaled_dev": (I, [P, I, P, P, P, P, P, I, F, P, P, P, U64, P, Z, P, P, P, P, F,
                                     F, I, I, P]),
    "nsm_adamw_tail_dev": (I, [P, P, P, P, P, P, P, I, P, P, P, P, D, D, D, D, P]),
    "nsm_adam_tail_dev": (I, [P, P, P, P, P, P, P, I, P, P, P, P, D, D, D, D, P]),
    "nsm_sgd_tail_dev": (I, [P, P, P, P, P, P, I, P, P, P, P, D, D, P]),
    "nsm_nchw_to_nhwc": (I, [P, I, I, I, I, P, I, I, I, P]),
    "nsm_nhwc_to_nchw": (I, [P, I, I, I, I, I, P, I, P]),
    "nsm_range_flag": (I, [P, L, F, F, P, P]),
    "nsm_dropout_masks": (I, [P, I, I, U64, P, P]),
    "nsm_dropout_masks_dev": (I, [P, I, I, P, P, P]),
    "nsm_stage_mark": (I, [I, P]),
# ... 58 lines not shown
```

### pcss-unet_amd/nsm_amd/ops.py

```python
import os

import torch

from ._lib import call, ptr, stream

F32 = torch.float32
BF16 = torch.bfloat16
F16S = torch.int16
PACK_FWD, PACK_DGRAD = 0, 1
NSM_F32, NSM_BF16, NSM_F16 = 0, 1, 2
S16 = (BF16, F16S)


def dt(t):
    if t.dtype == BF16:
        return NSM_BF16
    if t.dtype == F16S:
        return NSM_F16
    if t.dtype != F32:
        raise TypeError(f"activations must be float32, bfloat16 or f16 storage (int16), "
                        f"got {t.dtype}")
    return NSM_F32


# ... 397 lines not shown
    c_p = y.shape[1]
    n = (tile + 2) ** 2 * wino_tiles(B, H, W, tile) * 2 * c_p
    Vd = torch.empty(n, dtype=H2, device=y.device)
    dM = torch.empty(n, dtype=H2, device=y.device)
    call("nsm_wino_dual_input_bn_h2", ptr(d.g), d.g.stride(0), ptr(y), y.stride(0), B, H, W, c_p,
         tile, ptr(st.scale), ptr(st.shift), slope, ptr(mask), ptr(st.mean), ptr(d.coef), ptr(Vd),
         ptr(dM), ptr(bound), stream())
    return Vd, dM


def wino_dual_bn_f16(d, y, st, mask, B, H, W, bound, slope=0.2):
    c_p = y.shape[1]
    n = 36 * wino_tiles(B, H, W, 4) * c_p
    V = torch.empty(n, dtype=H2, device=y.device)
    dM = torch.empty(n, dtype=H2, device=y.device)
    call("nsm_wino_dual_bn_f16", ptr(d.g), d.g.stride(0), ptr(y), y.stride(0), B, H, W, c_p, 4,
         ptr(st.scale), ptr(st.shift), slope, ptr(mask), ptr(st.mean), ptr(d.coef), ptr(V), ptr(dM),
         ptr(bound), stream())
    return V, dM


def conv3x3_wgrad_wino(dy, V, B, H, W, cin_p, cin, cout, dw, tile=4, tag=None, dM=None,
                       amax=(None, None)):
    from ._lib import lib
    cout_p = dy.shape[1]
    ev = _probe(tag)
    if dM is not None and dM.dtype == H2:
        assert V.dtype == H2 and amax[0] is not None and amax[1] is not None
        n = int(lib.nsm_wino_wgrad_h2_ws(B, H, W, cin_p, cout_p, tile))
        ws = empty(n, device=dy.device)
        call("nsm_conv3x3_wgrad_wino_h2", ptr(dM), ptr(V), B, H, W, cin_p, cout_p, cin, cout,
             tile, ptr(dw), ptr(ws), n, ptr(amax[0]), ptr(amax[1]), stream())
        if ev is not None:
            ev.record()
        return
    n = int(lib.nsm_wino_wgrad_ws(B, H, W, cin_p, cout_p, tile))
    ws = empty(n, device=dy.device)
    if dM is None:
        call("nsm_conv3x3_wgrad_wino", ptr(dy), dy.stride(0), ptr(V), B, H, W, cin_p, cout_p, cin,
             cout, tile, ptr(dw), ptr(ws), n, stream())
    else:
        both = amax[0] is not None and amax[1] is not None
        call("nsm_conv3x3_wgrad_wino_dm", ptr(dM), ptr(V), B, H, W, cin_p, cout_p, cin, cout,
             tile, ptr(dw), ptr(ws), n, ptr(amax[0]) if both else None,
             ptr(amax[1]) if both else None, stream())
    if ev is not None:
        ev.record()


def conv_wgrad(dy, x, B, H, W, ksize, cin, cout, dw, pro=None, tag=None, amax=(None, None)):
    from ._lib import lib
    cout_p, cin_p = dy.shape[1], x.shape[1]
    bf = dy.dtype in S16
    if x.dtype != dy.dtype:
        raise TypeError("conv_wgrad: dy and x must share a dtype")
    n = int((lib.nsm_conv_wgrad_bf16_ws if bf else lib.nsm_conv_wgrad_ws)(B, H, W, cin_p, cout_p,
                                                                           ksize))
    ws = empty(max(n, 1), device=dy.device)
    sc = sh = mk = None
    if pro is not None:
        sc, sh, mk = pro
    ev = _probe(tag)
    args = (ptr(dy), dy.stride(0), ptr(x), x.stride(0), B, H, W, cin_p, cout_p, ksize, ptr(sc),
            ptr(sh), ptr(mk), 0.2, ptr(ws), n, cin, cout, ptr(dw))
    if bf:
        call("nsm_conv_wgrad_bf16" if dy.dtype == BF16 else "nsm_conv_wgrad_f16", *args, stream())
    else:
        call("nsm_conv_wgrad", *args, *_pair(amax), stream())
    if ev is not None:
        ev.record()


def call_ws(B, H, W, cin_p, cout_p, ksize):
    from ._lib import lib
    return lib.nsm_conv_wgrad_ws(B, H, W, cin_p, cout_p, ksize)


def reduce_chunks(M, C):
    from ._lib import lib
    return lib.nsm_reduce_chunks(M, C)


class BNState:
    __slots__ = ("scale", "shift", "mean", "invstd", "part", "nchunk", "gamma", "beta")

    def __init__(self, C, device):
        self.scale = empty(C, device=device)
        self.shift = empty(C, device=device)
        self.mean = empty(C, device=device)
        self.invstd = empty(C, device=device)
        self.part = None
        self.nchunk = 0
        self.gamma = None
        self.beta = None


def bn_partials(y):
    from ._lib import lib
    M, C = y.shape
    nchunk, rpc = reduce_chunks(M, C), lib.nsm_reduce_rows(M, C)
    part = Partials(empty(nchunk * 2 * C, device=y.device), nchunk, rpc)
    call("nsm_bn_stats", ptr(y), y.stride(0), M, C, ptr(part.buf), nchunk, dt(y), stream())
    return part


MERGE_ABOVE = int(os.environ.get("NSM_MERGE_ABOVE", "1024"))


def merged(part, M, C):
    if part.nchunk <= MERGE_ABOVE:
        return part
    if part._merged is None:
        G = -(-part.nchunk // MERGE_ABOVE)
        n2 = -(-part.nchunk // G)
        buf = empty(n2 * (2 if part.rpc else 3) * C, device=part.buf.device)
        call("nsm_bn_partials_merge", ptr(part.buf), part.nchunk, part.rpc, M, C, G, ptr(buf),
             stream())
        part._merged = Partials(buf, n2, part.rpc * G)
    return part._merged


def _finalize(part, M, C, bn_mod, c_real, momentum, eps, n_updates, st, gamma, beta=None,
              bound=None):
    part = merged(part, M, C)
    if beta is None:
        beta = pad_vec(bn_mod.bias.detach(), C)
    track = bn_mod.track_running_stats
    slot, mul = bound if bound is not None else (None, 1.0)
    call("nsm_bn_finalize_train", ptr(part.buf), part.nchunk, part.rpc, M, C, c_real, ptr(gamma),
         ptr(beta), ptr(bn_mod.running_mean if track else None),
         ptr(bn_mod.running_var if track else None),
         ptr(bn_mod.num_batches_tracked if track else None), momentum, eps, n_updates,
         ptr(st.mean), ptr(st.invstd), ptr(st.scale), ptr(st.shift), ptr(slot), float(mul),
         stream())


def bn_train(y, bn_mod, c_real, momentum, eps, n_updates=1, part=None, gamma=None, beta=None,
             bound=None):
    M, C = y.shape
    if part is None:
        part = bn_partials(y)
    st = BNState(C, y.device)
    st.part, st.nchunk = part, part.nchunk
    st.gamma = gamma if gamma is not None else pad_vec(bn_mod.weight.detach(), C)
    st.beta = beta if beta is not None else pad_vec(bn_mod.bias.detach(), C)
    _finalize(part, M, C, bn_mod, c_real, momentum, eps, n_updates, st, st.gamma, st.beta,
              bound=bound)
    return st


def bn_running_update(st, M, C, bn_mod, c_real, momentum, eps, n_updates=1):
    scratch = BNState(C, st.part.buf.device)
    _finalize(st.part, M, C, bn_mod, c_real, momentum, eps, n_updates, scratch, st.gamma, st.beta)


def bn_eval(bn_mod, C, c_real, eps, device, gamma=None, beta=None):
    st = BNState(C, device)
    st.gamma = gamma if gamma is not None else pad_vec(bn_mod.weight.detach(), C)
    beta = beta if beta is not None else pad_vec(bn_mod.bias.detach(), C)
    st.beta = beta
    bn_eval_into(st, bn_mod, C, c_real, eps)
    return st


def bn_eval_into(st, bn_mod, C, c_real, eps):
    call("nsm_bn_finalize_eval", ptr(bn_mod.running_mean), ptr(bn_mod.running_var), ptr(st.gamma),
         ptr(st.beta), C, c_real, eps, ptr(st.mean), ptr(st.invstd), ptr(st.scale), ptr(st.shift),
         stream())


def bn_act(y, st, slope=0.2, res=None, out=None, mask=None, HW=0, amax=None):
    M, C = y.shape
    o = out if out is not None else like(M, C, y)
    assert res is None or res.dtype == y.dtype
    assert mask is None or HW > 0
    call("nsm_bn_act", ptr(y), y.stride(0), M, C, ptr(st.scale), ptr(st.shift), slope, ptr(mask),
         HW, ptr(res), res.stride(0) if res is not None else 0, ptr(o), o.stride(0), dt(y),
         ptr(amax), stream())
    return o


def bn_act_h2(y, st, slope=0.2, mask=None, HW=0, bound=None):
    M, C = y.shape
    assert y.dtype == F32 and bound is not None and (mask is None or HW > 0)
    o = torch.empty(M, 2 * C, dtype=H2, device=y.device)
    call("nsm_bn_act_h2", ptr(y), y.stride(0), M, C, ptr(st.scale), ptr(st.shift), slope,
         ptr(mask), HW, ptr(o), ptr(bound), stream())
    return o


def to_h2(x, amax, beta=1.0):
    rows, C = x.shape
    assert x.is_contiguous() and x.dtype == F32
    o = torch.empty(rows, 2 * C, dtype=H2, device=x.device)
    call("nsm_to_h2", ptr(x), rows, C, ptr(amax), float(beta), ptr(o), stream())
    return o


def conv1x1_h2(xh, wh, bias, cout_p, stats=True, amax=(None, None), tag=None):
    from ._lib import lib
    M, cin2 = xh.shape
    assert xh.dtype == H2 and wh.dtype == H2 and amax[0] is not None and amax[1] is not None
    y = empty(M, cout_p, device=xh.device)
    part = None
    if stats:
        rpc = int(lib.nsm_conv1x1_h2_rows(M, cout_p, cin2, 0))
        nchunk = -(-M // rpc)
        part = Partials(empty(nchunk * 2 * cout_p, device=xh.device), nchunk, rpc)
    ev = _probe(tag)
    call("nsm_conv1x1_h2", ptr(xh), M, cin2 // 2, ptr(wh), ptr(bias), cout_p, ptr(y), y.stride(0),
         ptr(part.buf) if part is not None else None, ptr(amax[0]), ptr(amax[1]), stream())
    if ev is not None:
        ev.record()
    return y, part


def conv1x1_wgrad_h2(dyh, xh, cin, cout, dw, amax=(None, None), tag=None):
    from ._lib import lib
    M, cout2 = dyh.shape
    cin_p, cout_p = xh.shape[1] // 2, cout2 // 2
    assert xh.shape[0] == M and dyh.dtype == H2 and xh.dtype == H2
    n = int(lib.nsm_conv1x1_wgrad_h2_ws(M, cin_p, cout_p))
    ws = empty(max(n, 1), device=dyh.device)
    ev = _probe(tag)
    call("nsm_conv1x1_wgrad_h2", ptr(dyh), ptr(xh), M, cin_p, cout_p, cin, cout, ptr(dw), ptr(ws),
         n, ptr(amax[0]), ptr(amax[1]), stream())
    if ev is not None:
        ev.record()


def bn_bwd(g, y, st, HW, mask, c_real, dgamma, dbeta, dbias_prev, slope=0.2, part=None,
           defer=False, amax=None, h2=None):
    M, C = y.shape
    assert g.dtype == y.dtype
    k1dz, bound = h2 if h2 is not None else (None, None)
    if part is None:
        nchunk = reduce_chunks(M, C)
        partial = empty(nchunk * 2 * C, device=y.device)
        call("nsm_bn_bwd_reduce", ptr(g), g.stride(0), ptr(y), y.stride(0), M, C, HW,
             ptr(st.scale), ptr(st.shift), slope, ptr(mask), ptr(st.mean), ptr(st.invstd),
             ptr(partial), nchunk, dt(y), ptr(k1dz), stream())
    else:
        partial, nchunk = part
        if nchunk > SUM_ROWS_ABOVE:
            G = -(-nchunk // SUM_ROWS_ABOVE)
            n2 = -(-nchunk // G)
            buf = empty(n2 * 2 * C, device=y.device)
            call("nsm_sum_rows", ptr(partial), nchunk, 2 * C, G, ptr(buf), stream())
            partial, nchunk = buf, n2
    coef = empty(3 * C, device=y.device)
    call("nsm_bn_bwd_finalize", ptr(partial), nchunk, M, C, c_real, ptr(st.gamma), ptr(st.invstd),
         ptr(dgamma), ptr(dbeta), ptr(dbias_prev), ptr(coef), ptr(k1dz), ptr(bound), stream())
    if defer:
        return DeferredBnBwd(g, coef)
    if h2 is not None:
        assert y.dtype == F32
        dyh = torch.empty(M, 2 * C, dtype=H2, device=y.device)
        call("nsm_bn_bwd_apply_h2", ptr(g), g.stride(0), ptr(y), y.stride(0), M, C, HW,
             ptr(st.scale), ptr(st.shift), slope, ptr(mask), ptr(st.mean), ptr(coef), ptr(dyh),
             ptr(bound), stream())
        return dyh
    dy = like(M, C, y)
    call("nsm_bn_bwd_apply", ptr(g), g.stride(0), ptr(y), y.stride(0), M, C, HW, ptr(st.scale),
         ptr(st.shift), slope, ptr(mask), ptr(st.mean), ptr(coef), ptr(dy), dy.stride(0), dt(y),
         ptr(amax), stream())
    return dy


SUM_ROWS_ABOVE = int(os.environ.get("NSM_SUM_ROWS_ABOVE", "512"))


def conv1x1_dgrad_bn_bwd(dY2, B, H, W, w2d, y, st, mask, c_real, dgamma, dbeta, dbias_prev,
                         recompute, slope=0.2, tag=None, defer=False, amax=(None, None),
                         amax_out=None, bound=None):
    from ._lib import lib
    M, cop = dY2.shape
    C = y.shape[1]
    if dY2.dtype != y.dtype or w2d.dtype != y.dtype:
        raise TypeError("conv1x1_dgrad_bn_bwd: dY2, packed weight and Y1 must share a dtype")
    dtc = dt(y)
    nchunk = int(lib.nsm_conv1x1_bnbwd_chunks(B, H, W, C, cop, dtc))
    partial = empty(nchunk * 2 * C, device=y.device)
    dA1 = None if recompute else like(M, C, y)
    args = (ptr(dY2), dY2.stride(0), B, H, W, cop, ptr(w2d), C, ptr(y), y.stride(0),
            ptr(st.scale), ptr(st.shift), ptr(st.mean), ptr(st.invstd), ptr(mask), slope)
    ev = _probe(tag)
    am = _pair(amax) if dtc == NSM_F32 else (None, None)
    k1dz, bslot = bound if bound is not None else (None, None)
    assert bound is None or (dtc != NSM_F32 and not recompute)
    call("nsm_conv1x1_dgrad_bnbwd", *args, 0 if recompute else 1, ptr(partial), None, ptr(dA1),
         dA1.stride(0) if dA1 is not None else 0, dtc, *am, ptr(k1dz), stream())
    if nchunk > SUM_ROWS_ABOVE:
        G = -(-nchunk // SUM_ROWS_ABOVE)
        n2 = -(-nchunk // G)
        buf = empty(n2 * 2 * C, device=y.device)
        call("nsm_sum_rows", ptr(partial), nchunk, 2 * C, G, ptr(buf), stream())
        partial, nchunk = buf, n2
    coef = empty(3 * C, device=y.device)
    call("nsm_bn_bwd_finalize", ptr(partial), nchunk, M, C, c_real, ptr(st.gamma), ptr(st.invstd),
         ptr(dgamma), ptr(dbeta), ptr(dbias_prev), ptr(coef), ptr(k1dz), ptr(bslot), stream())
    if defer and not recompute:
        if ev is not None:
            ev.record()
        return DeferredBnBwd(dA1, coef)
    dy = like(M, C, y)
    if recompute:
        call("nsm_conv1x1_dgrad_bnbwd", *args, 2, None, ptr(coef), ptr(dy), dy.stride(0), dtc,
             *am, ptr(amax_out) if dtc == NSM_F32 else None, stream())
    else:
        call("nsm_bn_bwd_apply", ptr(dA1), dA1.stride(0), ptr(y), y.stride(0), M, C, H * W,
             ptr(st.scale), ptr(st.shift), slope, ptr(mask), ptr(st.mean), ptr(coef), ptr(dy),
             dy.stride(0), dtc, ptr(amax_out), stream())
    if ev is not None:
        ev.record()
    return dy


def conv1x1_dgrad_bn_bwd_h2(dY2h, HW, w2dh, y, st, mask, c_real, dgamma, dbeta, dbias_prev,
                            recompute, slope=0.2, tag=None, amax=(None, None), amax_out=None,
                            h2_out=None, defer=False):
    assert h2_out is None or not recompute
    assert not defer or h2_out is not None
    k1dz, bound = h2_out if h2_out is not None else (None, None)
    from ._lib import lib
    M, cop2 = dY2h.shape
    C = y.shape[1]
    assert dY2h.dtype == H2 and w2dh.dtype == H2 and y.dtype == F32
    nchunk = -(-M // int(lib.nsm_conv1x1_h2_rows(M, C, cop2, 1)))
    partial = empty(nchunk * 2 * C, device=y.device)
    dA1 = None if recompute else like(M, C, y)
    args = (ptr(dY2h), M, cop2 // 2, ptr(w2dh), C, ptr(y), y.stride(0), ptr(st.scale),
            ptr(st.shift), ptr(st.mean), ptr(st.invstd), ptr(mask), HW, slope)
    ev = _probe(tag)
    call("nsm_conv1x1_dgrad_bnbwd_h2", *args, 0 if recompute else 1, ptr(partial), None, ptr(dA1),
         dA1.stride(0) if dA1 is not None else 0, ptr(amax[0]), ptr(amax[1]), None, ptr(k1dz),
         stream())
    if nchunk > SUM_ROWS_ABOVE:
        G = -(-nchunk // SUM_ROWS_ABOVE)
        n2 = -(-nchunk // G)
        buf = empty(n2 * 2 * C, device=y.device)
        call("nsm_sum_rows", ptr(partial), nchunk, 2 * C, G, ptr(buf), stream())
        partial, nchunk = buf, n2
    coef = empty(3 * C, device=y.device)
    call("nsm_bn_bwd_finalize", ptr(partial), nchunk, M, C, c_real, ptr(st.gamma), ptr(st.invstd),
         ptr(dgamma), ptr(dbeta), ptr(dbias_prev), ptr(coef), ptr(k1dz), ptr(bound), stream())
    if defer:
        if ev is not None:
            ev.record()
        return DeferredBnBwd(dA1, coef)
    if h2_out is not None:
        dyh = torch.empty(M, 2 * C, dtype=H2, device=y.device)
        call("nsm_bn_bwd_apply_h2", ptr(dA1), dA1.stride(0), ptr(y), y.stride(0), M, C, HW,
             ptr(st.scale), ptr(st.shift), slope, ptr(mask), ptr(st.mean), ptr(coef), ptr(dyh),
             ptr(bound), stream())
        if ev is not None:
            ev.record()
        return dyh
    dy = like(M, C, y)
    if recompute:
        call("nsm_conv1x1_dgrad_bnbwd_h2", *args, 2, None, ptr(coef), ptr(dy), dy.stride(0),
             ptr(amax[0]), ptr(amax[1]), ptr(amax_out), None, stream())
    else:
        call("nsm_bn_bwd_apply", ptr(dA1), dA1.stride(0), ptr(y), y.stride(0), M, C, HW,
             ptr(st.scale), ptr(st.shift), slope, ptr(mask), ptr(st.mean), ptr(coef), ptr(dy),
             dy.stride(0), NSM_F32, ptr(amax_out), stream())
    if ev is not None:
        ev.record()
    return dy


def avgpool2(x, B, H, W):
    C = x.shape[1]
    y = like(B * (H // 2) * (W // 2), C, x)
    call("nsm_avgpool2_fwd", ptr(x), B, H, W, C, ptr(y), dt(x), stream())
    return y


def _bnred(kind, B, H, W, C, bnred, device, slope=0.2):
    from ._lib import lib
    if bnred is None:
        return None, None
    n = int(lib.nsm_bnred_chunks(kind, B, H, W, C))
    if n <= 0:
        return None, None
    y2, st = bnred[:2]
    k1dz = bnred[2] if len(bnred) > 2 else None
    partial = empty(n * 2 * C, device=device)
    return ((ptr(y2), ptr(st.scale), ptr(st.shift), ptr(st.mean), ptr(st.invstd), slope,
             ptr(partial), ptr(k1dz)), (partial, n))


def avgpool2_bwd_add(dy, B, H, W, skip, bnred=None):
    C = dy.shape[1]
    dx = like(B * H * W, C, dy)
    assert skip is None or skip.dtype == dy.dtype
    extra, part = _bnred(0, B, H, W, C, bnred, dy.device)
    if extra is None:
        call("nsm_avgpool2_bwd_add", ptr(dy), B, H, W, C, ptr(skip), ptr(dx), dt(dy), stream())
    else:
        call("nsm_avgpool2_bwd_add_bnred", ptr(dy), B, H, W, C, ptr(skip), ptr(dx), dt(dy),
             *extra, stream())
    return dx if bnred is None else (dx, part)


def resize(x, B, Hi, Wi, Ho, Wo):
    C = x.shape[-1]
    y = like(B * Ho * Wo, C, x)
    call("nsm_resize_fwd", ptr(x), B, Hi, Wi, C, ptr(y), Ho, Wo, dt(x), stream())
    return y


def resize_bwd(dy, B, Hi, Wi, Ho, Wo, bnred=None):
    C = dy.shape[-1]
    dx = like(B * Hi * Wi, C, dy)
    extra, part = _bnred(1, B, Hi, Wi, C, bnred, dy.device)
    if extra is None:
        call("nsm_resize_bwd", ptr(dy), B, Hi, Wi, C, ptr(dx), Ho, Wo, dt(dy), stream())
    else:
        call("nsm_resize_bwd_bnred", ptr(dy), B, Hi, Wi, C, ptr(dx), Ho, Wo, dt(dy), *extra,
             stream())
    return dx if bnred is None else (dx, part)


class Lazy:
    __slots__ = ("y2", "st", "res")

    def __init__(self, y2, st, res):
        self.y2, self.st, self.res = y2, st, res
# ... 19 lines not shown
         ptr(z.st.shift), slope, ptr(z.res), dt(z.y2), stream())
    return y


def bn_act_pool(y, st, B, H, W, slope=0.2, amax=None):
    C = y.shape[-1]
    z = like(B * H * W, C, y)
    pooled = like(B * (H // 2) * (W // 2), C, y)
    call("nsm_bn_act_pool", ptr(y), B, H, W, C, ptr(st.scale), ptr(st.shift), slope, ptr(z),
         ptr(pooled), dt(y), ptr(amax), stream())
    return z, pooled


def up2_resize(x, B, h, w, th, tw):
    C = x.shape[-1]
    y = like(B * th * tw, C, x)
    call("nsm_up2_resize_fwd", ptr(x), B, h, w, C, ptr(y), th, tw, dt(x), stream())
    return y


def up2_resize_bwd(dy, B, h, w, th, tw, bnred=None):
    C = dy.shape[-1]
    dx = like(B * h * w, C, dy)
    extra, part = _bnred(2, B, h, w, C, bnred, dy.device)
    if extra is None:
        call("nsm_up2_resize_bwd", ptr(dy), B, h, w, C, ptr(dx), th, tw, dt(dy), stream())
    else:
        call("nsm_up2_resize_bwd_bnred", ptr(dy), B, h, w, C, ptr(dx), th, tw, dt(dy), *extra,
             stream())
    return dx if bnred is None else (dx, part)


def input_prep(x, cp, dtype=F32, amax=None):
    B, C, H, W = x.shape
    out = torch.empty(B * (H // 2) * (W // 2), cp, dtype=dtype, device=x.device)
    call("nsm_input_prep", ptr(x), B, C, H, W, ptr(out), cp, dt(out),
         ptr(amax) if dtype == F32 else None, stream())
    return out


def input_prep_h2(x, cp, amax):
    B, C, H, W = x.shape
    out = torch.empty(B * (H // 2) * (W // 2), 2 * cp, dtype=H2, device=x.device)
    call("nsm_input_prep_h2", ptr(x), B, C, H, W, ptr(out), cp, ptr(amax), stream())
    return out


def conv3x3_h2(xh, B, H, W, wh, bias, cout_p, stats=True, amax=(None, None), tag=None):
    from ._lib import lib
    M, cin2 = xh.shape
    assert xh.dtype == H2 and wh.dtype == H2 and M == B * H * W
    y = empty(M, cout_p, device=xh.device)
    part = None
    if stats:
        rpc = int(lib.nsm_conv3x3_h2_rows(M, cout_p))
        part = Partials(empty(-(-M // rpc) * 2 * cout_p, device=xh.device), -(-M // rpc), rpc)
    ev = _probe(tag)
    call("nsm_conv3x3_h2", ptr(xh), B, H, W, cin2 // 2, ptr(wh), ptr(bias), cout_p, ptr(y),
         y.stride(0), ptr(part.buf) if part is not None else None, ptr(amax[0]), ptr(amax[1]),
         stream())
    if ev is not None:
        ev.record()
    return y, part


def conv3x3_wgrad_h2(dyh, xh, B, H, W, cin, cout, dw, amax=(None, None), tag=None):
    from ._lib import lib
    cin_p, cout_p = xh.shape[1] // 2, dyh.shape[1] // 2
    n = int(lib.nsm_conv3x3_wgrad_h2_ws(B, H, W, cin_p, cout_p))
    ws = empty(max(n, 1), device=dyh.device)
    ev = _probe(tag)
    call("nsm_conv3x3_wgrad_h2", ptr(dyh), ptr(xh), B, H, W, cin_p, cout_p, cin, cout, ptr(dw),
         ptr(ws), n, ptr(amax[0]), ptr(amax[1]), stream())
    if ev is not None:
        ev.record()


def input_grad(dX, B, C, H, W):
    dx = empty(B, C, H, W, device=dX.device)
    call("nsm_input_grad", ptr(dX), B, C, H, W, dX.shape[1], ptr(dx), dt(dX), stream())
    return dx


def head_fwd(z, B, Rh, Rw, w10, b10):
    out = empty(B, 1, 2 * Rh, 2 * Rw, device=z.device)
    call("nsm_head_fwd", ptr(z), z.stride(0), B, Rh, Rw, ptr(w10), ptr(b10), ptr(out), dt(z),
         stream())
    return out


def head_bwd(gout, out, z, B, Rh, Rw, w10, dw10, db10):
    from ._lib import lib
    nblk = lib.nsm_head_bwd_blocks(B, Rh, Rw)
    partial = empty(nblk * 68, device=z.device)
    dz = torch.empty(*z.shape, dtype=z.dtype, device=z.device)
    call("nsm_head_bwd", ptr(gout), ptr(out), ptr(z), z.stride(0), B, Rh, Rw, ptr(w10), ptr(dz),
         ptr(partial), ptr(dw10), ptr(db10), dt(z), stream())
    return dz


def vgg_prep(output, target, mean, denom):
    B, _, H, W = output.shape
    out = empty(2 * B * H * W, 32, device=output.device)
    call("nsm_vgg_prep", ptr(output), ptr(target), B, H, W, float(mean), float(denom), ptr(out),
         stream())
    return out


def maxpool2(x, B, H, W):
    C = x.shape[1]
    y = empty(B * (H // 2) * (W // 2), C, device=x.device)
    call("nsm_maxpool2_fwd", ptr(x), B, H, W, C, ptr(y), stream())
    return y


def vgg_tap_relu_bwd(g, y, t, coef, gscale, relu=True):
    n = y.numel()
    over = g is None
    if over:
        g = torch.empty_like(y)
    assert g.numel() == n and g.is_contiguous() and y.is_contiguous()
    assert t is None or (t.numel() == n and t.is_contiguous())
    call("nsm_vgg_tap_relu_bwd", ptr(g), ptr(y), ptr(t), n, float(coef), ptr(gscale), int(relu),
         int(over), stream())
    return g


def maxpool2_bwd(gp, y, t, B, H, W, coef, gscale):
    C = y.shape[1]
    assert y.shape[0] == B * H * W and gp.shape == (B * (H // 2) * (W // 2), C)
    assert y.is_contiguous() and gp.is_contiguous() and (t is None or (
        t.shape == y.shape and t.is_contiguous()))
    gy = empty(B * H * W, C, device=y.device)
    call("nsm_maxpool2_bwd", ptr(gp), ptr(y), ptr(t), B, H, W, C, float(coef), ptr(gscale),
         ptr(gy), stream())
    return gy


def vgg_prep_bwd(g32, output, denom, grad, scale=1.0, accumulate=False):
    B, _, H, W = output.shape
    assert g32.shape == (B * H * W, 32) and g32.is_contiguous()
    assert grad.numel() == B * H * W and grad.is_contiguous() and output.is_contiguous()
    call("nsm_vgg_prep_bwd", ptr(g32), ptr(output), B, H, W, float(denom), float(scale),
         ptr(grad), int(accumulate), stream())
    return grad


def l1_mean(a, b, alpha=1.0):
    from ._lib import lib
    n = a.numel()
    assert b.numel() == n and a.is_contiguous() and b.is_contiguous()
    partial = empty(int(lib.nsm_loss_blocks(n)), device=a.device)
    out = torch.empty((), dtype=F32, device=a.device)
    call("nsm_l1_loss_fwd", ptr(a), ptr(b), n, float(alpha), ptr(partial), ptr(out), stream())
    return out
```

### pcss-unet_amd/nsm_amd/unet.py

```python
import os
import warnings

import torch
import torch.distributed as dist
import torch.nn as nn

from . import ops, optim
from ._lib import call, ptr, require_gpu, stream
from . import prep
from .prep import H2_WINO, LazyBlockWeights, StepWeights

SLOPE = 0.2
WINOGRAD_MIN_CHANNELS = (int(os.environ.get("NSM_WINO_MIN", "64"))
                         if os.environ.get("NSM_WINOGRAD", "1") != "0" else 1 << 30)
LAZY_DECODER = os.environ.get("NSM_LAZY_DECODER", "0") != "0"
EVAL_FUSED = os.environ.get("NSM_EVAL_FUSED", "1") != "0"
_WINO_ENV = os.environ.get("NSM_WINO_TILE", "")
WINO_TILE = int(_WINO_ENV) if _WINO_ENV else 4


def wino_tile(cin_p, H, W):
    if _WINO_ENV:
        return int(_WINO_ENV)
    f6 = 64 * -(-H // 6) * -(-W // 6)
# ... 732 lines not shown
    @staticmethod
    def forward(ctx, x, mod, *params):
        training = mod.training
        B, C, H, W = x.shape
        dev = x.device
        x32 = x.detach().to(torch.float32)
        orig_hw = (H, W)
        if H % 2 or W % 2:
            He, We = H - H % 2, W - W % 2
            x32 = ops.resize(x32.contiguous().view(B * C * H * W, 1), B * C, H, W, He, We).view(B, C, He, We)
            H, W = He, We
        x32 = x32.contiguous()
        Rh, Rw = H // 2, W // 2
        cin_p = ops.pad32(4 * C)
        assert mod.conv2.conv[0].in_channels == 4 * C, (
            f"Unet expects {mod.conv2.conv[0].in_channels // 4} input channels, got {C}")
        cdt = mod.activation_dtype()
        masks, mask_max = _masks_for(mod, B, dev, training)
        amax = torch.empty(AM_PER_BLOCK * 10 * ops.AMAX_WORDS, dtype=torch.int32, device=dev)
        sw = _step_weights(mod, cdt, Rh, Rw, training, act_slots=amax)
        w1_2 = (sw.block(2).w1(ops.PACK_FWD)
                if ops.pad32(mod.conv2.conv[0].in_channels) < WINOGRAD_MIN_CHANNELS else None)
        if w1_2 is not None and w1_2.dtype == ops.H2:
            X = ops.input_prep_h2(x32, cin_p, _x_slot(amax, 2))
        else:
            X = ops.input_prep(x32, cin_p, cdt, amax=_x_slot(amax, 2))

        saved, c, shapes = {}, {}, {}
        inp, h, w = X, Rh, Rw
        for k in ENCODER:
            with ops.stage(f"conv{k}.fwd"):
                s = _block_fwd(mod.block(k), inp, B, h, w, training, masks.get(k), f"conv{k}",
                               pw=sw.block(k), fuse_out=True,
                               am=_block_slots(amax, k), mask_max=mask_max.get(k, 1.0))
                saved[k], shapes[k] = s, (h, w)
                if s.Z is not None:
                    c[k] = s.Z
                    if k < 5:
                        inp = ops.avgpool2(c[k], B, h, w)
                elif k < 5:
                    c[k], inp = ops.bn_act_pool(s.Y2, s.bn2, B, h, w, SLOPE,
                                                amax=_x_slot(amax, k + 1))
                elif LAZY_DECODER and cdt == torch.bfloat16:
                    c[k] = ops.Lazy(s.Y2, s.bn2, None)
                else:
                    c[k] = ops.bn_act(s.Y2, s.bn2, SLOPE, amax=_x_slot(amax, k + 1))
                if k < 5:
                    h, w = h // 2, w // 2
        skip_shape = {6: shapes[4], 7: shapes[3], 8: shapes[2], 9: (Rh, Rw)}
        cur, (h, w) = c[5], shapes[5]
        ups = {}
        for k in DECODER:
            with ops.stage(f"conv{k}.fwd"):
                h2, w2 = 2 * h, 2 * w
                th, tw = skip_shape[k]
                src = None
                lazy = isinstance(cur, ops.Lazy)
                if (th, tw) != (h2, w2):
                    up = ops.up2_resize_act(cur, B, h, w, th, tw, SLOPE) if lazy else None
                    if up is None:
                        cur = cur.materialise(SLOPE) if lazy else cur
                        up = ops.up2_resize(cur, B, h, w, th, tw)
                elif fuses_resize(mod.block(k), cdt, training):
                    if lazy:
                        cur = cur.materialise(SLOPE)
                        ops.absmax(cur, _x_slot(amax, k))
                    up, src = None, (cur, h, w)
                elif lazy:
                    up = ops.resize_act(cur, B, h, w, h2, w2, SLOPE)
                else:
                    up = ops.resize(cur, B, h, w, h2, w2)
                if lazy and up is not None:
                    ops.absmax(up, _x_slot(amax, k))
                ups[k] = (h, w, h2, w2, th, tw)
                res = c[SKIP_OF[k]] if k in SKIP_OF else None
                s = _block_fwd(mod.block(k), up, B, th, tw, training, masks.get(k), f"conv{k}",
                               pw=sw.block(k), src=src, fuse_out=True, res=res,
                               am=_block_slots(amax, k), mask_max=mask_max.get(k, 1.0))
                saved[k] = s
                if s.Z is not None:
                    cur = s.Z
                elif k != 9 and LAZY_DECODER and cdt == torch.bfloat16:
                    cur = ops.Lazy(s.Y2, s.bn2, res)
                else:
                    cur = ops.bn_act(s.Y2, s.bn2, SLOPE, res=res,
                                     amax=_x_slot(amax, k + 1) if k < 9 else None)
                h, w = th, tw
        z9 = cur
        with ops.stage("head.fwd"):
            out = ops.head_fwd(z9, B, Rh, Rw, mod.conv10.weight.detach(), mod.conv10.bias.detach())

        if _FROZEN is not None and not training:
            _FROZEN.ready = True
        if training:
            for bm in mod.modules():
                if isinstance(bm, nn.BatchNorm2d):
                    for b in (bm.running_mean, bm.running_var, bm.num_batches_tracked):
                        torch.autograd.graph.increment_version(b)
        ctx.mod = mod
        ctx.saved_blocks = saved
        ctx.ups = ups
        ctx.meta = (B, C, H, W, orig_hw, Rh, Rw, training)
        ctx.z9 = z9
        ctx.save_for_backward(out)
        ctx.params = params
        return out

    @staticmethod
    def backward(ctx, gout):
        mod = ctx.mod
        (out,) = ctx.saved_tensors
        B, C, H, W, orig_hw, Rh, Rw, training = ctx.meta
        if not training:
            raise RuntimeError("nsm_amd Unet backward is implemented for train mode (as the "
                               "reference trains); eval-mode BN backward is not on the hot path")
        params = ctx.params
        dev = out.device
        total = sum(p.numel() for p in params)
        flat = torch.empty(total, dtype=torch.float32, device=dev)
        grads, off = {}, 0
        views, offset_of = [], {}
        for p in params:
            v = flat[off:off + p.numel()].view_as(p)
            grads[p] = v
            views.append(v)
            offset_of[id(p)] = off
            off += p.numel()
        dp = mod._grad_allreduce
        split = offset_of.get(id(mod.conv6.conv[0].weight)) if dp is not None else None
        global _wg_stream
        side = None
        if WGRAD_STREAM and not (GRAPH_SIDE_F32 == 0 and torch.cuda.is_current_stream_capturing()
                                 and ctx.saved_blocks[2].Y1.dtype == torch.float32):
            side = _wg_streams.get(dev)
            if side is None:
                side = _wg_streams[dev] = torch.cuda.Stream(device=dev)
        _wg_stream = side
        try:
            return _UnetFn._backward(ctx, gout, mod, out, params, flat, grads, views, dp, split)
        finally:
            _wg_stream = None
            if side is not None:
                torch.cuda.current_stream().wait_stream(side)
            _wg_hold.clear()

    @staticmethod
    def _backward(ctx, gout, mod, out, params, flat, grads, views, dp, split):
        B, C, H, W, orig_hw, Rh, Rw, training = ctx.meta
        total = flat.numel()

        gout = gout.contiguous().to(torch.float32)
        with ops.stage("head.bwd"):
            G = ops.head_bwd(gout, out, ctx.z9, B, Rh, Rw, mod.conv10.weight.detach(),
                             grads[mod.conv10.weight], grads[mod.conv10.bias])
        sb = ctx.saved_blocks
        skip_grad = {}
        gpart = None
        for k in (9, 8, 7, 6):
            s = sb[k]
            with ops.stage(f"conv{k}.bwd"):
                dX = _block_bwd(mod.block(k), s, G, grads, True, f"conv{k}", gpart=gpart)
                h, w, h2, w2, th, tw = ctx.ups[k]
                if (th, tw) != (h2, w2):
                    dprev, gpart = ops.up2_resize_bwd(dX, B, h, w, th, tw), None
                else:
                    dprev, gpart = ops.resize_bwd(dX, B, h, w, h2, w2, bnred=_bnred_of(sb[k - 1]))
            if k - 1 in SKIP_OF:
                skip_grad[SKIP_OF[k - 1]] = dprev
            G = dprev
        if split is not None:
            _allreduce_bucket(flat, split, total, dp[0])
        need_x = ctx.needs_input_grad[0]
        for k in (5, 4, 3, 2):
            s = sb[k]
            st = ops.stage(f"conv{k}.bwd")
            st.__enter__()
            dX = _block_bwd(mod.block(k), s, G, grads, need_dx=(k > 2 or need_x), name=f"conv{k}",
                            gpart=gpart)
            if k == 5 and training and mod.emulate_checkpoint_bn:
                blk = mod.block(5)
                M = s.B * s.H * s.W
                ops.bn_running_update(s.bn1, M, s.cip, blk.conv[1], blk.conv[0].in_channels,
                                      blk.conv[1].momentum, blk.conv[1].eps)
                ops.bn_running_update(s.bn2, M, s.cop, blk.conv[5], blk.conv[4].out_channels,
                                      blk.conv[5].momentum, blk.conv[5].eps)
            if k > 2:
                ph, pw = sb[k - 1].H, sb[k - 1].W
                G, gpart = ops.avgpool2_bwd_add(dX, B, ph, pw, skip_grad.get(k - 1),
                                                bnred=_bnred_of(sb[k - 1]))
            else:
                G = dX
            st.__exit__(None, None, None)
        if split is not None:
            _allreduce_bucket(flat, 0, split, dp[0])
        dx = None
        if need_x:
            dx = ops.input_grad(G, B, C, H, W)
            if (H, W) != tuple(orig_hw):
                H0, W0 = orig_hw
                dx = ops.resize_bwd(dx.view(B * C * H * W, 1), B * C, H0, W0, H, W).view(B, C, H0, W0)
        ctx.saved_blocks = None
        ctx.z9 = None
        return (dx, None) + tuple(views)
```

Measured before the change: 780.8 frames/s.

## Fuse final BN+LReLU into head conv and merge BN finalize reductions

```diff
diff --git a/include/nsm.h b/include/nsm.h
--- a/include/nsm.h
+++ b/include/nsm.h
@@ -190,6 +190,12 @@
                           float bound_mul, void* stream);
 int nsm_bn_partials_merge(const float* partial, int nchunk, int rows_per_chunk, int M, int C,
                           int group, float* out, void* stream);
+int nsm_bn_finalize_train_rows(const float* partial, int nchunk, int rows_per_chunk, int M, int C,
+                               int c_real, int group, float* merged, uint32_t* ticket,
+                               const float* gamma, const float* beta, float* run_mean,
+                               float* run_var, int64_t* num_batches, float momentum, float eps,
+                               int n_updates, float* mean, float* invstd, float* scale,
+                               float* shift, uint32_t* bound, float bound_mul, void* stream);
 int nsm_bn_finalize_eval(const float* run_mean, const float* run_var, const float* gamma,
                          const float* beta, int C, int c_real, float eps, float* mean,
                          float* invstd, float* scale, float* shift, void* stream);
@@ -208,6 +214,11 @@
                         float* dbias_prev, float* coef, const uint32_t* amax_k1dz,
                         uint32_t* bound, void* stream);
 int nsm_sum_rows(const float* part, int nrows, int width, int group, float* out, void* stream);
+int nsm_bn_bwd_finalize_rows(const float* partial, int nchunk, int M, int C, int c_real, int group,
+                             float* summed, uint32_t* ticket, const float* gamma,
+                             const float* invstd, float* dgamma, float* dbeta, float* dbias_prev,
+                             float* coef, const uint32_t* amax_k1dz, uint32_t* bound,
+                             void* stream);
 int nsm_bn_bwd_apply(const void* g, int ldg, const void* y, int ldy, int M, int C, int HW,
                      const float* scale, const float* shift, float slope, const float* mask,
                      const float* mean, const float* coef, void* dy, int lddy, int dtype,
@@ -264,6 +275,14 @@
 int nsm_head_bwd(const float* gout, const float* out, const void* z, int ldz, int B, int Rh,
                  int Rw, const float* w10, void* dz, float* partial, float* dw10, float* db10,
                  int dtype, void* stream);
+int nsm_head_fwd_bn(const void* y2, int ldy, int B, int Rh, int Rw, const float* scale,
+                    const float* shift, float slope, const float* w10, const float* b10,
+                    float* out, int dtype, void* stream);
+int nsm_head_bwd_bn(const float* gout, const float* out, const void* y2, int ldy, int B, int Rh,
+                    int Rw, const float* scale, const float* shift, const float* mean,
+                    const float* invstd, float slope, const float* w10, void* dz, float* partial,
+                    float* bn_partial, uint32_t* amax_k1dz, float* dw10, float* db10, int dtype,
+                    void* stream);
 
 int nsm_loss_blocks(int64_t n);
 int nsm_l1_loss_fwd(const float* o, const float* t, int64_t n, float alpha, float* partial,
diff --git a/pcss-unet_amd/csrc/nsm_elem.hip b/pcss-unet_amd/csrc/nsm_elem.hip
--- a/pcss-unet_amd/csrc/nsm_elem.hip
+++ b/pcss-unet_amd/csrc/nsm_elem.hip
@@ -86,39 +86,51 @@
   return (red[0] + red[1]) + (red[2] + red[3]);
 }
 
-__global__ void __launch_bounds__(256) bn_finalize_train_kernel(
-    const float* __restrict__ partial, int nchunk, int rpc, int M, int C, int c_real,
-    const float* __restrict__ gamma, const float* __restrict__ beta, float* run_mean,
-    float* run_var, int64_t* num_batches, float momentum, float eps, int n_updates, float* mean_o,
-    float* invstd_o, float* scale_o, float* shift_o, uint32_t* bound, float bound_mul) {
-  __shared__ double red[4];
+struct RowsGlobal {
+  const float* p;
+  size_t st;
+  int C, c;
+  __device__ __forceinline__ float operator()(int k, int v) const { return p[k * st + v * C + c]; }
+};
+template <int NV, int CS>
+struct RowsLds {
+  const float* p;
+  int j;
+  __device__ __forceinline__ float operator()(int k, int v) const {
+    return p[(k * NV + v) * CS + j];
+  }
+};
+
+template <typename R>
+__device__ __forceinline__ void bn_finalize_train_body(
+    const R& rows, int c, int nchunk, int rpc, int M, int c_real, const float* __restrict__ gamma,
+    const float* __restrict__ beta, float* run_mean, float* run_var, float momentum, float eps,
+    int n_updates, float* mean_o, float* invstd_o, float* scale_o, float* shift_o, uint32_t* bound,
+    float bound_mul, double* red) {
   const int tid = threadIdx.x;
-  const int c = blockIdx.x;
-  if (blockIdx.x == 0 && tid == 0 && num_batches) *num_batches += n_updates;
-  const size_t st = (size_t)(rpc ? 2 : 3) * C;
   double s0 = 0.0, s1 = 0.0, s2 = 0.0, s3 = 0.0;
   int k = tid;
   for (; k + 768 < nchunk; k += 1024) {
-    s0 += partial[k * st + c];
-    s1 += partial[(k + 256) * st + c];
-    s2 += partial[(k + 512) * st + c];
-    s3 += partial[(k + 768) * st + c];
-  }
-  for (; k < nchunk; k += 256) s0 += partial[k * st + c];
+    s0 += rows(k, 0);
+    s1 += rows(k + 256, 0);
+    s2 += rows(k + 512, 0);
+    s3 += rows(k + 768, 0);
+  }
+  for (; k < nchunk; k += 256) s0 += rows(k, 0);
   const double mean = block_sum_d((s0 + s1) + (s2 + s3), red) / M;
   double q0 = 0.0, q1 = 0.0;
   for (k = tid; k < nchunk; k += 512) {
-    int n0 = rpc ? min(M, k * rpc + rpc) - k * rpc : (int)partial[k * st + 2 * C + c];
+    int n0 = rpc ? min(M, k * rpc + rpc) - k * rpc : (int)rows(k, 2);
     if (n0 > 0) {
-      double d = partial[k * st + c] / n0 - mean;
-      q0 += partial[k * st + C + c] + n0 * d * d;
+      double d = rows(k, 0) / n0 - mean;
+      q0 += rows(k, 1) + n0 * d * d;
     }
     int k1 = k + 256;
     if (k1 < nchunk) {
-      int n1 = rpc ? min(M, k1 * rpc + rpc) - k1 * rpc : (int)partial[k1 * st + 2 * C + c];
+      int n1 = rpc ? min(M, k1 * rpc + rpc) - k1 * rpc : (int)rows(k1, 2);
       if (n1 > 0) {
-        double d = partial[k1 * st + c] / n1 - mean;
-        q1 += partial[k1 * st + C + c] + n1 * d * d;
+        double d = rows(k1, 0) / n1 - mean;
+        q1 += rows(k1, 1) + n1 * d * d;
       }
     }
   }
@@ -149,11 +161,22 @@
   }
 }
 
-__global__ void bn_partials_merge_kernel(const float* __restrict__ partial, int nchunk, int rpc,
-                                         int M, int C, int G, float* __restrict__ out) {
-  const int c = blockIdx.x * blockDim.x + threadIdx.x;
-  const int g = blockIdx.y;
-  if (c >= C) return;
+__global__ void __launch_bounds__(256) bn_finalize_train_kernel(
+    const float* __restrict__ partial, int nchunk, int rpc, int M, int C, int c_real,
+    const float* __restrict__ gamma, const float* __restrict__ beta, float* run_mean,
+    float* run_var, int64_t* num_batches, float momentum, float eps, int n_updates, float* mean_o,
+    float* invstd_o, float* scale_o, float* shift_o, uint32_t* bound, float bound_mul) {
+  __shared__ double red[4];
+  const int c = blockIdx.x;
+  if (blockIdx.x == 0 && threadIdx.x == 0 && num_batches) *num_batches += n_updates;
+  bn_finalize_train_body(RowsGlobal{partial, (size_t)(rpc ? 2 : 3) * C, C, c}, c, nchunk, rpc, M,
+                         c_real, gamma, beta, run_mean, run_var, momentum, eps, n_updates, mean_o,
+                         invstd_o, scale_o, shift_o, bound, bound_mul, red);
+}
+
+__device__ __forceinline__ void bn_merge_group(const float* __restrict__ partial, int nchunk,
+                                               int rpc, int M, int C, int G, int g, int c,
+                                               float* __restrict__ out) {
   const size_t st = (size_t)(rpc ? 2 : 3) * C;
   const int k0 = g * G, k1 = min(nchunk, k0 + G);
   double s = 0.0;
@@ -174,11 +197,16 @@
   out[(size_t)g * st + C + c] = (float)m2;
   if (!rpc) out[(size_t)g * st + 2 * C + c] = (float)n;
 }
-
-__global__ void sum_rows_kernel(const float* __restrict__ part, int nrows, int width, int G,
-                                float* __restrict__ out) {
-  const int j = blockIdx.x * blockDim.x + threadIdx.x, g = blockIdx.y;
-  if (j >= width) return;
+__global__ void bn_partials_merge_kernel(const float* __restrict__ partial, int nchunk, int rpc,
+                                         int M, int C, int G, float* __restrict__ out) {
+  const int c = blockIdx.x * blockDim.x + threadIdx.x;
+  if (c >= C) return;
+  bn_merge_group(partial, nchunk, rpc, M, C, G, blockIdx.y, c, out);
+}
+
+__device__ __forceinline__ void sum_rows_group(const float* __restrict__ part, int nrows,
+                                               int width, int G, int g, int j,
+                                               float* __restrict__ out) {
   const int k0 = g * G, k1 = min(nrows, k0 + G);
   double s = 0.0, s1 = 0.0;
   int k = k0;
@@ -188,6 +216,62 @@
   }
   if (k < k1) s += part[(size_t)k * width + j];
   out[(size_t)g * width + j] = (float)(s + s1);
+}
+__global__ void sum_rows_kernel(const float* __restrict__ part, int nrows, int width, int G,
+                                float* __restrict__ out) {
+  const int j = blockIdx.x * blockDim.x + threadIdx.x;
+  if (j >= width) return;
+  sum_rows_group(part, nrows, width, G, blockIdx.y, j, out);
+}
+
+constexpr int FIN_CS = 4;
+constexpr int FIN_FWD_ROWS = 1024;
+constexpr int FIN_BWD_ROWS = 512;
+
+__device__ __forceinline__ bool slice_ticket_last(uint32_t* ticket, int* flag) {
+  __threadfence();
+  __syncthreads();
+  if (threadIdx.x == 0) {
+    const uint32_t t = atomicAdd(ticket + blockIdx.x, 1u);
+    const int last = t == gridDim.y - 1;
+    if (last) atomicExch(ticket + blockIdx.x, 0u);
+    *flag = last;
+  }
+  __syncthreads();
+  const bool last = *flag != 0;
+  if (last) __threadfence();
+  return last;
+}
+__device__ __forceinline__ float ld_coherent(const float* p) {
+  return __hip_atomic_load(p, __ATOMIC_RELAXED, __HIP_MEMORY_SCOPE_AGENT);
+}
+
+__global__ void __launch_bounds__(256) bn_finalize_train_rows_kernel(
+    const float* __restrict__ partial, int nchunk, int rpc, int M, int C, int c_real, int G, int n2,
+    float* buf, uint32_t* ticket, const float* __restrict__ gamma, const float* __restrict__ beta,
+    float* run_mean, float* run_var, int64_t* num_batches, float momentum, float eps, int n_updates,
+    float* mean_o, float* invstd_o, float* scale_o, float* shift_o, uint32_t* bound,
+    float bound_mul) {
+  __shared__ float rows[FIN_FWD_ROWS * 3 * FIN_CS];
+  __shared__ double red[4];
+  __shared__ int flag;
+  const int tid = threadIdx.x, j = tid & (FIN_CS - 1);
+  const int c0 = blockIdx.x * FIN_CS;
+  const int g = blockIdx.y * (256 / FIN_CS) + tid / FIN_CS;
+  if (g < n2) bn_merge_group(partial, nchunk, rpc, M, C, G, g, c0 + j, buf);
+  if (!slice_ticket_last(ticket, &flag)) return;
+  const int nv = rpc ? 2 : 3;
+  const size_t st = (size_t)nv * C;
+  for (int i = tid; i < n2 * nv * FIN_CS; i += 256) {
+    const int jj = i & (FIN_CS - 1), kv = i / FIN_CS, k = kv / nv, v = kv - k * nv;
+    rows[(k * 3 + v) * FIN_CS + jj] = ld_coherent(buf + (size_t)k * st + v * C + c0 + jj);
+  }
+  __syncthreads();
+  if (blockIdx.x == 0 && tid == 0 && num_batches) *num_batches += n_updates;
+  for (int jj = 0; jj < FIN_CS; ++jj)
+    bn_finalize_train_body(RowsLds<3, FIN_CS>{rows, jj}, c0 + jj, n2, rpc * G, M, c_real, gamma,
+                           beta, run_mean, run_var, momentum, eps, n_updates, mean_o, invstd_o,
+                           scale_o, shift_o, bound, bound_mul, red);
 }
 
 __global__ void bn_finalize_eval_kernel(const float* __restrict__ rm, const float* __restrict__ rv,
@@ -214,6 +298,10 @@
   return F8{lrelu4(v.a, slope), lrelu4(v.b, slope)};
 }
 
+__device__ __forceinline__ F8 bn_lrelu8(F8 y, F8 sc, F8 sh, float slope) {
+  return lrelu8(y * sc + sh, slope);
+}
+
 template <typename T>
 __global__ void __launch_bounds__(256) bn_act_kernel(const T* __restrict__ y, int ldy, int M,
                                                      int C8, FastDiv fdHW,
@@ -229,7 +317,7 @@
   const int pstep = gridDim.x * ppb;
   uint32_t am = 0;
   for (int p = blockIdx.x * ppb + tp; p < M; p += pstep) {
-    F8 o = lrelu8(ld8(y + (size_t)p * ldy + c) * sc + sh, slope);
+    F8 o = bn_lrelu8(ld8(y + (size_t)p * ldy + c), sc, sh, slope);
     if (mask) o = o * ld8(mask + (size_t)fdiv((uint32_t)p, fdHW) * (C8 * 8) + c);
     if (res) o += ld8(res + (size_t)p * ldres + c);
     st8(out + (size_t)p * ldo + c, o);
@@ -314,27 +402,24 @@
   }
 }
 
-__global__ void __launch_bounds__(256) bn_bwd_finalize_kernel(
-    const float* __restrict__ partial, int nchunk, int M, int C, int c_real,
-    const float* __restrict__ gamma, const float* __restrict__ invstd, float* dgamma,
-    float* dbeta, float* dbias_prev, float* coef, const uint32_t* __restrict__ amax_k1dz,
-    uint32_t* __restrict__ bound) {
-  __shared__ double red[4];
+template <typename R>
+__device__ __forceinline__ void bn_bwd_finalize_body(
+    const R& rows, int c, int nchunk, int M, int C, int c_real, const float* __restrict__ gamma,
+    const float* __restrict__ invstd, float* dgamma, float* dbeta, float* dbias_prev, float* coef,
+    const uint32_t* __restrict__ amax_k1dz, uint32_t* __restrict__ bound, double* red) {
   const int tid = threadIdx.x;
-  const int c = blockIdx.x;
   const float a_k1dz = bound ? __uint_as_float(amax_read(amax_k1dz)) : 0.f;
-  const size_t st = (size_t)2 * C;
   double a0 = 0.0, a1 = 0.0, b0 = 0.0, b1 = 0.0;
   int k = tid;
   for (; k + 256 < nchunk; k += 512) {
-    a0 += partial[k * st + c];
-    b0 += partial[k * st + C + c];
-    a1 += partial[(k + 256) * st + c];
-    b1 += partial[(k + 256) * st + C + c];
+    a0 += rows(k, 0);
+    b0 += rows(k, 1);
+    a1 += rows(k + 256, 0);
+    b1 += rows(k + 256, 1);
   }
   for (; k < nchunk; k += 256) {
-    a0 += partial[k * st + c];
-    b0 += partial[k * st + C + c];
+    a0 += rows(k, 0);
+    b0 += rows(k, 1);
   }
   const double S1 = block_sum_d(a0 + a1, red), S2 = block_sum_d(b0 + b1, red);
   if (tid != 0) return;
@@ -356,6 +441,40 @@
     if (dbeta) dbeta[c] = (float)S1;
     if (dbias_prev) dbias_prev[c] = (float)((double)k1 * S1 + (double)k3 * M);
   }
+}
+
+__global__ void __launch_bounds__(256) bn_bwd_finalize_kernel(
+    const float* __restrict__ partial, int nchunk, int M, int C, int c_real,
+    const float* __restrict__ gamma, const float* __restrict__ invstd, float* dgamma,
+    float* dbeta, float* dbias_prev, float* coef, const uint32_t* __restrict__ amax_k1dz,
+    uint32_t* __restrict__ bound) {
+  __shared__ double red[4];
+  const int c = blockIdx.x;
+  bn_bwd_finalize_body(RowsGlobal{partial, (size_t)2 * C, C, c}, c, nchunk, M, C, c_real, gamma,
+                       invstd, dgamma, dbeta, dbias_prev, coef, amax_k1dz, bound, red);
+}
+
+__global__ void __launch_bounds__(256) bn_bwd_finalize_rows_kernel(
+    const float* __restrict__ partial, int nchunk, int M, int C, int c_real, int G, int n2,
+    float* buf, uint32_t* ticket, const float* __restrict__ gamma,
+    const float* __restrict__ invstd, float* dgamma, float* dbeta, float* dbias_prev, float* coef,
+    const uint32_t* __restrict__ amax_k1dz, uint32_t* __restrict__ bound) {
+  __shared__ float rows[FIN_BWD_ROWS * 2 * FIN_CS];
+  __shared__ double red[4];
+  __shared__ int flag;
+  const int tid = threadIdx.x, j = tid & (FIN_CS - 1), v = (tid / FIN_CS) & 1;
+  const int c0 = blockIdx.x * FIN_CS;
+  const int g = blockIdx.y * (128 / FIN_CS) + tid / (2 * FIN_CS);
+  if (g < n2) sum_rows_group(partial, nchunk, 2 * C, G, g, v * C + c0 + j, buf);
+  if (!slice_ticket_last(ticket, &flag)) return;
+  for (int i = tid; i < n2 * 2 * FIN_CS; i += 256) {
+    const int jj = i & (FIN_CS - 1), kv = i / FIN_CS, k = kv >> 1, vv = kv & 1;
+    rows[i] = ld_coherent(buf + (size_t)k * 2 * C + vv * C + c0 + jj);
+  }
+  __syncthreads();
+  for (int jj = 0; jj < FIN_CS; ++jj)
+    bn_bwd_finalize_body(RowsLds<2, FIN_CS>{rows, jj}, c0 + jj, n2, M, C, c_real, gamma, invstd,
+                         dgamma, dbeta, dbias_prev, coef, amax_k1dz, bound, red);
 }
 
 template <typename T>
@@ -447,7 +566,9 @@
   }
   template <typename T>
   __device__ void add(const BnRedP& r, F8 g, size_t p, int C, int c) {
-    const F8 v = ld8((const T*)r.y + p * C + c);
+    add_v(r, g, ld8((const T*)r.y + p * C + c), C, c);
+  }
+  __device__ void add_v(const BnRedP& r, F8 g, F8 v, int C, int c) {
     const F8 dz = bn_dz8(g, v, sc, sh, r.slope, nullptr, 0, C, c);
     s1 += dz;
     s2 += dz * ((v - mu) * is);
@@ -1397,22 +1518,41 @@
   }
 }
 
-template <typename T>
+template <typename T, bool BN = false>
 __global__ void head_fwd_kernel(const T* __restrict__ z, int ldz, int B, int Rh, int Rw,
                                 const float* __restrict__ w10, const float* __restrict__ b10,
-                                float* __restrict__ out) {
+                                float* __restrict__ out, const float* __restrict__ scale,
+                                const float* __restrict__ shift, float slope) {
   __shared__ float w[68];
   if (threadIdx.x < 64) w[threadIdx.x] = w10[threadIdx.x];
   if (threadIdx.x < 4) w[64 + threadIdx.x] = b10[threadIdx.x];
   __syncthreads();
+  F8 sc0, sc1, sh0, sh1;
+  if constexpr (BN) {
+    sc0 = ldf8(scale);
+    sc1 = ldf8(scale + 8);
+    sh0 = ldf8(shift);
+    sh1 = ldf8(shift + 8);
+  }
   long long npix = (long long)B * Rh * Rw;
   for (long long p = (long long)blockIdx.x * blockDim.x + threadIdx.x; p < npix;
        p += (long long)gridDim.x * blockDim.x) {
     float zz[16];
     const T* zr = z + (size_t)p * ldz;
+    f32x4 zq[4];
+#pragma unroll
+    for (int q = 0; q < 4; ++q) zq[q] = ld4(zr + 4 * q);
+    if constexpr (BN) {
+      const F8 z0 = as_stored8<T>(bn_lrelu8(F8{zq[0], zq[1]}, sc0, sh0, slope));
+      const F8 z1 = as_stored8<T>(bn_lrelu8(F8{zq[2], zq[3]}, sc1, sh1, slope));
+      zq[0] = z0.a;
+      zq[1] = z0.b;
+      zq[2] = z1.a;
+      zq[3] = z1.b;
+    }
 #pragma unroll
     for (int q = 0; q < 4; ++q) {
-      f32x4 v = ld4(zr + 4 * q);
+      const f32x4 v = zq[q];
       zz[4 * q] = v.x;
       zz[4 * q + 1] = v.y;
       zz[4 * q + 2] = v.z;
@@ -1441,11 +1581,11 @@
   return v;
 }
 
-template <typename T>
+template <typename T, bool BN = false>
 __global__ void __launch_bounds__(256) head_bwd_kernel(
     const float* __restrict__ gout, const float* __restrict__ out, const T* __restrict__ z,
     int ldz, int B, int Rh, int Rw, const float* __restrict__ w10, T* __restrict__ dz,
-    float* __restrict__ partial) {
+    float* __restrict__ partial, BnRedP rp) {
   __shared__ float w[64];
   __shared__ float red[4][68];
   if (threadIdx.x < 64) w[threadIdx.x] = w10[threadIdx.x];
@@ -1453,6 +1593,11 @@
   float accw[68];
 #pragma unroll
   for (int k = 0; k < 68; ++k) accw[k] = 0.f;
+  BnRedAcc ra0, ra1;
+  if constexpr (BN) {
+    ra0.init(rp, 0);
+    ra1.init(rp, 8);
+  }
   long long npix = (long long)B * Rh * Rw;
   for (long long p = (long long)blockIdx.x * blockDim.x + threadIdx.x; p < npix;
        p += (long long)gridDim.x * blockDim.x) {
@@ -1470,16 +1615,30 @@
     }
     const T* zr = z + (size_t)p * ldz;
     T* dzr = dz + (size_t)p * ldz;
+    f32x4 zq[4], gq[4];
+#pragma unroll
+    for (int q = 0; q < 4; ++q) zq[q] = ld4(zr + 4 * q);
+    F8 y0, y1;
+    if constexpr (BN) {
+      y0 = F8{zq[0], zq[1]};
+      y1 = F8{zq[2], zq[3]};
+      const F8 z0 = as_stored8<T>(bn_lrelu8(y0, ra0.sc, ra0.sh, rp.slope));
+      const F8 z1 = as_stored8<T>(bn_lrelu8(y1, ra1.sc, ra1.sh, rp.slope));
+      zq[0] = z0.a;
+      zq[1] = z0.b;
+      zq[2] = z1.a;
+      zq[3] = z1.b;
+    }
 #pragma unroll
     for (int q = 0; q < 4; ++q) {
-      f32x4 v = ld4(zr + 4 * q);
+      const f32x4 v = zq[q];
       float zv[4] = {v.x, v.y, v.z, v.w};
       f32x4 g;
       float gv[4];
 #pragma unroll
       for (int e = 0; e < 4; ++e) {
         int c = 4 * q + e;
-        gv[e] = d[0] * w[c] + d[1] * w[16 + c] + d[2] * w[32 + c] + d[3] * w[48 + c];
+        gv[e] = fmaf(d[3], w[48 + c], fmaf(d[2], w[32 + c], fmaf(d[0], w[c], d[1] * w[16 + c])));
 #pragma unroll
         for (int j = 0; j < 4; ++j) accw[j * 16 + c] += d[j] * zv[e];
       }
@@ -1488,6 +1647,11 @@
       g.z = gv[2];
       g.w = gv[3];
       st4(dzr + 4 * q, g);
+      gq[q] = g;
+    }
+    if constexpr (BN) {
+      ra0.add_v(rp, as_stored8<T>(F8{gq[0], gq[1]}), y0, ldz, 0);
+      ra1.add_v(rp, as_stored8<T>(F8{gq[2], gq[3]}), y1, ldz, 8);
     }
     for (int c = 16; c < ldz; c += 4) st4(dzr + c, f32x4{0.f, 0.f, 0.f, 0.f});
 #pragma unroll
@@ -1513,6 +1677,28 @@
   if (threadIdx.x < 68) {
     float s = red[0][threadIdx.x] + red[1][threadIdx.x] + red[2][threadIdx.x] + red[3][threadIdx.x];
     partial[(size_t)blockIdx.x * 68 + threadIdx.x] = s;
+  }
+  if constexpr (BN) {
+    __shared__ float redb[4][32];
+    const F8 acc[4] = {ra0.s1, ra1.s1, ra0.s2, ra1.s2};
+#pragma unroll
+    for (int i = 0; i < 4; ++i) {
+      const float e[8] = {acc[i].a.x, acc[i].a.y, acc[i].a.z, acc[i].a.w,
+                          acc[i].b.x, acc[i].b.y, acc[i].b.z, acc[i].b.w};
+#pragma unroll
+      for (int k = 0; k < 8; ++k) {
+        const float s = wave_sum(e[k]);
+        if (lane == 0) redb[wv][8 * i + k] = s;
+      }
+    }
+    __syncthreads();
+    const int t = threadIdx.x;
+    if (t < 2 * ldz) {
+      const int which = t >= ldz, c = t - which * ldz, k = which * 16 + c;
+      const float s = c < 16 ? (redb[0][k] + redb[1][k]) + (redb[2][k] + redb[3][k]) : 0.f;
+      rp.partial[(size_t)blockIdx.x * 2 * ldz + t] = s;
+    }
+    amax_flush(max(ra0.am, ra1.am), rp.amax);
   }
 }
 
@@ -1804,6 +1990,32 @@
                      run_var, num_batches, momentum, eps, n_updates, mean, invstd, scale, shift,
                      bound, bound_mul);
   NSM_LAUNCH_CHECK("bn_finalize_train");
+  return 0;
+}
+
+extern "C" int nsm_bn_finalize_train_rows(const float* partial, int nchunk, int rows_per_chunk,
+                                          int M, int C, int c_real, int group, float* merged,
+                                          uint32_t* ticket, const float* gamma, const float* beta,
+                                          float* run_mean, float* run_var, int64_t* num_batches,
+                                          float momentum, float eps, int n_updates, float* mean,
+                                          float* invstd, float* scale, float* shift,
+                                          uint32_t* bound, float bound_mul, void* stream) {
+  NSM_CHECK_ARG(partial && merged && ticket && gamma && beta && mean && invstd && scale && shift,
+                "bn_finalize_train_rows: null");
+  NSM_CHECK_ARG(M > 1, "bn_finalize: Expected more than 1 value per channel when training");
+  NSM_CHECK_ARG(nchunk >= 1 && group >= 1 && C >= FIN_CS && C % FIN_CS == 0 &&
+                    (rows_per_chunk == 0 ||
+                     (rows_per_chunk >= 1 && (long long)nchunk * rows_per_chunk >= M)),
+                "bn_finalize_train_rows: bad args");
+  const int n2 = ceil_div(nchunk, group);
+  NSM_CHECK_ARG(n2 <= FIN_FWD_ROWS && (long long)rows_per_chunk * group < (1ll << 31),
+                "bn_finalize_train_rows: more than 1024 merged rows");
+  const dim3 grid(C / FIN_CS, ceil_div(n2, 256 / FIN_CS));
+  hipLaunchKernelGGL(bn_finalize_train_rows_kernel, grid, dim3(256), 0, as_stream(stream), partial,
+                     nchunk, rows_per_chunk, M, C, c_real, group, n2, merged, ticket, gamma, beta,
+                     run_mean, run_var, num_batches, momentum, eps, n_updates, mean, invstd, scale,
+                     shift, bound, bound_mul);
+  NSM_LAUNCH_CHECK("bn_finalize_train_rows");
   return 0;
 }
 
@@ -1933,6 +2145,27 @@
                      as_stream(stream), partial, nchunk, M, C, c_real, gamma, invstd, dgamma, dbeta,
                      dbias_prev, coef, amax_k1dz, bound);
   NSM_LAUNCH_CHECK("bn_bwd_finalize");
+  return 0;
+}
+
+extern "C" int nsm_bn_bwd_finalize_rows(const float* partial, int nchunk, int M, int C, int c_real,
+                                        int group, float* summed, uint32_t* ticket,
+                                        const float* gamma, const float* invstd, float* dgamma,
+                                        float* dbeta, float* dbias_prev, float* coef,
+                                        const uint32_t* amax_k1dz, uint32_t* bound, void* stream) {
+  NSM_CHECK_ARG(partial && summed && ticket && gamma && invstd && coef,
+                "bn_bwd_finalize_rows: bad args");
+  NSM_CHECK_ARG(!bound || amax_k1dz, "bn_bwd_finalize: a bound needs the max|k1 dz| slot");
+  NSM_CHECK_ARG(M > 1 || !bound, "bn_bwd_finalize: M");
+  NSM_CHECK_ARG(nchunk >= 1 && group >= 1 && C >= FIN_CS && C % FIN_CS == 0,
+                "bn_bwd_finalize_rows: bad args");
+  const int n2 = ceil_div(nchunk, group);
+  NSM_CHECK_ARG(n2 <= FIN_BWD_ROWS, "bn_bwd_finalize_rows: more than 512 summed rows");
+  const dim3 grid(C / FIN_CS, ceil_div(n2, 128 / FIN_CS));
+  hipLaunchKernelGGL(bn_bwd_finalize_rows_kernel, grid, dim3(256), 0, as_stream(stream), partial,
+                     nchunk, M, C, c_real, group, n2, summed, ticket, gamma, invstd, dgamma, dbeta,
+                     dbias_prev, coef, amax_k1dz, bound);
+  NSM_LAUNCH_CHECK("bn_bwd_finalize_rows");
   return 0;
 }
 
@@ -2437,19 +2670,55 @@
   dim3 g(grid_for(npix));
   if (dtype == NSM_BF16)
     hipLaunchKernelGGL(head_fwd_kernel<bf16_t>, g, dim3(256), 0, as_stream(stream),
-                       NSM_CT(bf16_t, z), ldz, B, Rh, Rw, w10, b10, out);
+                       NSM_CT(bf16_t, z), ldz, B, Rh, Rw, w10, b10, out, nullptr, nullptr, 0.f);
   else if (dtype == NSM_F16)
     hipLaunchKernelGGL(head_fwd_kernel<f16_t>, g, dim3(256), 0, as_stream(stream),
-                       NSM_CT(f16_t, z), ldz, B, Rh, Rw, w10, b10, out);
+                       NSM_CT(f16_t, z), ldz, B, Rh, Rw, w10, b10, out, nullptr, nullptr, 0.f);
   else
     hipLaunchKernelGGL(head_fwd_kernel<float>, g, dim3(256), 0, as_stream(stream),
-                       NSM_CT(float, z), ldz, B, Rh, Rw, w10, b10, out);
+                       NSM_CT(float, z), ldz, B, Rh, Rw, w10, b10, out, nullptr, nullptr, 0.f);
   NSM_LAUNCH_CHECK("head_fwd");
+  return 0;
+}
+
+extern "C" int nsm_head_fwd_bn(const void* y2, int ldy, int B, int Rh, int Rw, const float* scale,
+                               const float* shift, float slope, const float* w10,
+                               const float* b10, float* out, int dtype, void* stream) {
+  NSM_CHECK_ARG(y2 && scale && shift && w10 && b10 && out && ldy >= 16 && ldy % 4 == 0,
+                "head_fwd_bn: bad args");
+  NSM_CHECK_ARG(dtype == NSM_F32, "head_fwd_bn: fp32 only");
+  long long npix = (long long)B * Rh * Rw;
+  dim3 g(grid_for(npix));
+  hipLaunchKernelGGL((head_fwd_kernel<float, true>), g, dim3(256), 0, as_stream(stream),
+                     (const float*)y2, ldy, B, Rh, Rw, w10, b10, out, scale, shift, slope);
+  NSM_LAUNCH_CHECK("head_fwd_bn");
   return 0;
 }
 
 extern "C" int nsm_head_bwd_blocks(int B, int Rh, int Rw) {
   return grid_for((long long)B * Rh * Rw, 256, 1024);
+}
+
+extern "C" int nsm_head_bwd_bn(const float* gout, const float* out, const void* y2, int ldy, int B,
+                               int Rh, int Rw, const float* scale, const float* shift,
+                               const float* mean, const float* invstd, float slope,
+                               const float* w10, void* dz, float* partial, float* bn_partial,
+                               uint32_t* amax_k1dz, float* dw10, float* db10, int dtype,
+                               void* stream) {
+  NSM_CHECK_ARG(gout && out && y2 && w10 && dz && partial && dw10 && db10 && scale && shift &&
+                    mean && invstd && bn_partial,
+                "head_bwd_bn: bad args");
+  NSM_CHECK_ARG(ldy >= 16 && ldy % 8 == 0 && ldy <= 128, "head_bwd_bn: 16 <= ldy <= 128, ldy % 8 == 0");
+  NSM_CHECK_ARG(dtype == NSM_F32, "head_bwd_bn: fp32 only");
+  int nblk = nsm_head_bwd_blocks(B, Rh, Rw);
+  hipStream_t s = as_stream(stream);
+  const BnRedP rp{y2, scale, shift, mean, invstd, slope, bn_partial, amax_k1dz};
+  hipLaunchKernelGGL((head_bwd_kernel<float, true>), dim3(nblk), dim3(256), 0, s, gout, out,
+                     (const float*)y2, ldy, B, Rh, Rw, w10, (float*)dz, partial, rp);
+  NSM_LAUNCH_CHECK("head_bwd_bn");
+  hipLaunchKernelGGL(head_reduce_kernel, dim3(68), dim3(256), 0, s, partial, nblk, dw10, db10);
+  NSM_LAUNCH_CHECK("head_reduce");
+  return 0;
 }
 
 extern "C" int nsm_head_bwd(const float* gout, const float* out, const void* z, int ldz, int B,
@@ -2461,13 +2730,13 @@
   hipStream_t s = as_stream(stream);
   if (dtype == NSM_BF16)
     hipLaunchKernelGGL(head_bwd_kernel<bf16_t>, dim3(nblk), dim3(256), 0, s, gout, out,
-                       NSM_CT(bf16_t, z), ldz, B, Rh, Rw, w10, NSM_T(bf16_t, dz), partial);
+                       NSM_CT(bf16_t, z), ldz, B, Rh, Rw, w10, NSM_T(bf16_t, dz), partial, BnRedP{});
   else if (dtype == NSM_F16)
     hipLaunchKernelGGL(head_bwd_kernel<f16_t>, dim3(nblk), dim3(256), 0, s, gout, out,
-                       NSM_CT(f16_t, z), ldz, B, Rh, Rw, w10, NSM_T(f16_t, dz), partial);
+                       NSM_CT(f16_t, z), ldz, B, Rh, Rw, w10, NSM_T(f16_t, dz), partial, BnRedP{});
   else
     hipLaunchKernelGGL(head_bwd_kernel<float>, dim3(nblk), dim3(256), 0, s, gout, out,
-                       NSM_CT(float, z), ldz, B, Rh, Rw, w10, NSM_T(float, dz), partial);
+                       NSM_CT(float, z), ldz, B, Rh, Rw, w10, NSM_T(float, dz), partial, BnRedP{});
   NSM_LAUNCH_CHECK("head_bwd");
   hipLaunchKernelGGL(head_reduce_kernel, dim3(68), dim3(256), 0, s, partial, nblk, dw10, db10);
   NSM_LAUNCH_CHECK("head_reduce");
diff --git a/pcss-unet_amd/nsm_amd/_lib.py b/pcss-unet_amd/nsm_amd/_lib.py
--- a/pcss-unet_amd/nsm_amd/_lib.py
+++ b/pcss-unet_amd/nsm_amd/_lib.py
@@ -75,6 +75,9 @@
     "nsm_conv1x1_wgrad_h2_ws": (Z, [I, I, I]),
     "nsm_conv1x1_wgrad_h2": (I, [P, P, I, I, I, I, I, P, P, Z, P, P, P]),
     "nsm_bn_partials_merge": (I, [P, I, I, I, I, I, P, P]),
+    "nsm_bn_finalize_train_rows": (I, [P, I, I, I, I, I, I, P, P, P, P, P, P, P, F, F, I, P, P, P, P,
+                                       P, F, P]),
+    "nsm_bn_bwd_finalize_rows": (I, [P, I, I, I, I, I, P, P, P, P, P, P, P, P, P, P, P]),
     "nsm_bn_finalize_eval": (I, [P, P, P, P, I, I, F, P, P, P, P, P]),
     "nsm_bn_act": (I, [P, I, I, I, P, P, F, P, I, P, I, P, I, I, P, P]),
     "nsm_bn_bwd_reduce": (I, [P, I, P, I, I, I, I, P, P, F, P, P, P, P, I, I, P, P]),
@@ -112,6 +115,8 @@
     "nsm_head_fwd": (I, [P, I, I, I, I, P, P, P, I, P]),
     "nsm_head_bwd_blocks": (I, [I, I, I]),
     "nsm_head_bwd": (I, [P, P, P, I, I, I, I, P, P, P, P, P, I, P]),
+    "nsm_head_fwd_bn": (I, [P, I, I, I, I, P, P, F, P, P, P, I, P]),
+    "nsm_head_bwd_bn": (I, [P, P, P, I, I, I, I, P, P, P, P, F, P, P, P, P, P, P, P, I, P]),
     "nsm_loss_blocks": (I, [L]),
     "nsm_l1_loss_fwd": (I, [P, P, L, F, P, P, P]),
     "nsm_expdiff_mean": (I, [P, P, L, F, P, P, P]),
diff --git a/pcss-unet_amd/nsm_amd/ops.py b/pcss-unet_amd/nsm_amd/ops.py
--- a/pcss-unet_amd/nsm_amd/ops.py
+++ b/pcss-unet_amd/nsm_amd/ops.py
@@ -503,7 +503,7 @@
 
 
 class BNState:
-    __slots__ = ("scale", "shift", "mean", "invstd", "part", "nchunk", "gamma", "beta")
+    __slots__ = ("scale", "shift", "mean", "invstd", "part", "nchunk", "gamma", "beta", "tickets")
 
     def __init__(self, C, device):
         self.scale = empty(C, device=device)
@@ -514,6 +514,7 @@
         self.nchunk = 0
         self.gamma = None
         self.beta = None
+        self.tickets = None
 
 
 def bn_partials(y):
@@ -541,13 +542,36 @@
     return part._merged
 
 
+FIN_FWD_ROWS, FIN_BWD_ROWS = 1024, 512
+
+
+def tickets(owner, C, device):
+    d = owner.__dict__
+    t = d.get("_nsm_tickets")
+    if t is None or t.numel() < C // 4 or t.device != device:
+        t = d["_nsm_tickets"] = torch.zeros(max(C // 4, 64), dtype=torch.int32, device=device)
+    return t
+
+
 def _finalize(part, M, C, bn_mod, c_real, momentum, eps, n_updates, st, gamma, beta=None,
               bound=None):
-    part = merged(part, M, C)
     if beta is None:
         beta = pad_vec(bn_mod.bias.detach(), C)
     track = bn_mod.track_running_stats
     slot, mul = bound if bound is not None else (None, 1.0)
+    if part.nchunk > MERGE_ABOVE and MERGE_ABOVE <= FIN_FWD_ROWS and C % 4 == 0:
+        G = -(-part.nchunk // MERGE_ABOVE)
+        n2 = -(-part.nchunk // G)
+        buf = empty(n2 * (2 if part.rpc else 3) * C, device=part.buf.device)
+        call("nsm_bn_finalize_train_rows", ptr(part.buf), part.nchunk, part.rpc, M, C, c_real, G,
+             ptr(buf), ptr(tickets(bn_mod, C, part.buf.device)), ptr(gamma), ptr(beta),
+             ptr(bn_mod.running_mean if track else None),
+             ptr(bn_mod.running_var if track else None),
+             ptr(bn_mod.num_batches_tracked if track else None), momentum, eps, n_updates,
+             ptr(st.mean), ptr(st.invstd), ptr(st.scale), ptr(st.shift), ptr(slot), float(mul),
+             stream())
+        return
+    part = merged(part, M, C)
     call("nsm_bn_finalize_train", ptr(part.buf), part.nchunk, part.rpc, M, C, c_real, ptr(gamma),
          ptr(beta), ptr(bn_mod.running_mean if track else None),
          ptr(bn_mod.running_var if track else None),
@@ -563,6 +587,7 @@
         part = bn_partials(y)
     st = BNState(C, y.device)
     st.part, st.nchunk = part, part.nchunk
+    st.tickets = tickets(bn_mod, C, y.device)
     st.gamma = gamma if gamma is not None else pad_vec(bn_mod.weight.detach(), C)
     st.beta = beta if beta is not None else pad_vec(bn_mod.bias.detach(), C)
     _finalize(part, M, C, bn_mod, c_real, momentum, eps, n_updates, st, st.gamma, st.beta,
@@ -663,15 +688,7 @@
              ptr(partial), nchunk, dt(y), ptr(k1dz), stream())
     else:
         partial, nchunk = part
-        if nchunk > SUM_ROWS_ABOVE:
-            G = -(-nchunk // SUM_ROWS_ABOVE)
-            n2 = -(-nchunk // G)
-            buf = empty(n2 * 2 * C, device=y.device)
-            call("nsm_sum_rows", ptr(partial), nchunk, 2 * C, G, ptr(buf), stream())
-            partial, nchunk = buf, n2
-    coef = empty(3 * C, device=y.device)
-    call("nsm_bn_bwd_finalize", ptr(partial), nchunk, M, C, c_real, ptr(st.gamma), ptr(st.invstd),
-         ptr(dgamma), ptr(dbeta), ptr(dbias_prev), ptr(coef), ptr(k1dz), ptr(bound), stream())
+    coef = _bwd_finalize(partial, nchunk, M, C, c_real, st, dgamma, dbeta, dbias_prev, k1dz, bound)
     if defer:
         return DeferredBnBwd(g, coef)
     if h2 is not None:
@@ -691,6 +708,27 @@
 SUM_ROWS_ABOVE = int(os.environ.get("NSM_SUM_ROWS_ABOVE", "512"))
 
 
+def _bwd_finalize(partial, nchunk, M, C, c_real, st, dgamma, dbeta, dbias_prev, k1dz, bound):
+    coef = empty(3 * C, device=partial.device)
+    if nchunk > SUM_ROWS_ABOVE:
+        G = -(-nchunk // SUM_ROWS_ABOVE)
+        n2 = -(-nchunk // G)
+        buf = empty(n2 * 2 * C, device=partial.device)
+        if SUM_ROWS_ABOVE <= FIN_BWD_ROWS and C % 4 == 0:
+            tk = getattr(st, "tickets", None)
+            if tk is None or tk.numel() < C // 4:
+                tk = torch.zeros(max(C // 4, 64), dtype=torch.int32, device=partial.device)
+            call("nsm_bn_bwd_finalize_rows", ptr(partial), nchunk, M, C, c_real, G, ptr(buf),
+                 ptr(tk), ptr(st.gamma), ptr(st.invstd), ptr(dgamma), ptr(dbeta),
+                 ptr(dbias_prev), ptr(coef), ptr(k1dz), ptr(bound), stream())
+            return coef
+        call("nsm_sum_rows", ptr(partial), nchunk, 2 * C, G, ptr(buf), stream())
+        partial, nchunk = buf, n2
+    call("nsm_bn_bwd_finalize", ptr(partial), nchunk, M, C, c_real, ptr(st.gamma), ptr(st.invstd),
+         ptr(dgamma), ptr(dbeta), ptr(dbias_prev), ptr(coef), ptr(k1dz), ptr(bound), stream())
+    return coef
+
+
 def conv1x1_dgrad_bn_bwd(dY2, B, H, W, w2d, y, st, mask, c_real, dgamma, dbeta, dbias_prev,
                          recompute, slope=0.2, tag=None, defer=False, amax=(None, None),
                          amax_out=None, bound=None):
@@ -711,15 +749,7 @@
     assert bound is None or (dtc != NSM_F32 and not recompute)
     call("nsm_conv1x1_dgrad_bnbwd", *args, 0 if recompute else 1, ptr(partial), None, ptr(dA1),
          dA1.stride(0) if dA1 is not None else 0, dtc, *am, ptr(k1dz), stream())
-    if nchunk > SUM_ROWS_ABOVE:
-        G = -(-nchunk // SUM_ROWS_ABOVE)
-        n2 = -(-nchunk // G)
-        buf = empty(n2 * 2 * C, device=y.device)
-        call("nsm_sum_rows", ptr(partial), nchunk, 2 * C, G, ptr(buf), stream())
-        partial, nchunk = buf, n2
-    coef = empty(3 * C, device=y.device)
-    call("nsm_bn_bwd_finalize", ptr(partial), nchunk, M, C, c_real, ptr(st.gamma), ptr(st.invstd),
-         ptr(dgamma), ptr(dbeta), ptr(dbias_prev), ptr(coef), ptr(k1dz), ptr(bslot), stream())
+    coef = _bwd_finalize(partial, nchunk, M, C, c_real, st, dgamma, dbeta, dbias_prev, k1dz, bslot)
     if defer and not recompute:
         if ev is not None:
             ev.record()
@@ -756,15 +786,7 @@
     call("nsm_conv1x1_dgrad_bnbwd_h2", *args, 0 if recompute else 1, ptr(partial), None, ptr(dA1),
          dA1.stride(0) if dA1 is not None else 0, ptr(amax[0]), ptr(amax[1]), None, ptr(k1dz),
          stream())
-    if nchunk > SUM_ROWS_ABOVE:
-        G = -(-nchunk // SUM_ROWS_ABOVE)
-        n2 = -(-nchunk // G)
-        buf = empty(n2 * 2 * C, device=y.device)
-        call("nsm_sum_rows", ptr(partial), nchunk, 2 * C, G, ptr(buf), stream())
-        partial, nchunk = buf, n2
-    coef = empty(3 * C, device=y.device)
-    call("nsm_bn_bwd_finalize", ptr(partial), nchunk, M, C, c_real, ptr(st.gamma), ptr(st.invstd),
-         ptr(dgamma), ptr(dbeta), ptr(dbias_prev), ptr(coef), ptr(k1dz), ptr(bound), stream())
+    coef = _bwd_finalize(partial, nchunk, M, C, c_real, st, dgamma, dbeta, dbias_prev, k1dz, bound)
     if defer:
         if ev is not None:
             ev.record()
@@ -950,18 +972,33 @@
     return dx
 
 
-def head_fwd(z, B, Rh, Rw, w10, b10):
+def head_fwd(z, B, Rh, Rw, w10, b10, bn=None, slope=0.2):
     out = empty(B, 1, 2 * Rh, 2 * Rw, device=z.device)
+    if bn is not None:
+        call("nsm_head_fwd_bn", ptr(z), z.stride(0), B, Rh, Rw, ptr(bn.scale), ptr(bn.shift), slope,
+             ptr(w10), ptr(b10), ptr(out), dt(z), stream())
+        return out
     call("nsm_head_fwd", ptr(z), z.stride(0), B, Rh, Rw, ptr(w10), ptr(b10), ptr(out), dt(z),
          stream())
     return out
 
 
-def head_bwd(gout, out, z, B, Rh, Rw, w10, dw10, db10):
+def head_bwd(gout, out, z, B, Rh, Rw, w10, dw10, db10, bnred=None, slope=0.2):
     from ._lib import lib
     nblk = lib.nsm_head_bwd_blocks(B, Rh, Rw)
-    partial = empty(nblk * 68, device=z.device)
-    dz = torch.empty(*z.shape, dtype=z.dtype, device=z.device)
+    src = z if bnred is None else bnred[0]
+    partial = empty(nblk * 68, device=src.device)
+    dz = torch.empty(*src.shape, dtype=src.dtype, device=src.device)
+    if bnred is not None:
+        y2, st = bnred[:2]
+        k1dz = bnred[2] if len(bnred) > 2 else None
+        C = y2.shape[1]
+        assert y2.stride(0) == C and st.scale.numel() == C
+        bpart = empty(nblk * 2 * C, device=y2.device)
+        call("nsm_head_bwd_bn", ptr(gout), ptr(out), ptr(y2), C, B, Rh, Rw, ptr(st.scale),
+             ptr(st.shift), ptr(st.mean), ptr(st.invstd), slope, ptr(w10), ptr(dz), ptr(partial),
+             ptr(bpart), ptr(k1dz), ptr(dw10), ptr(db10), dt(y2), stream())
+        return dz, (bpart, nblk)
     call("nsm_head_bwd", ptr(gout), ptr(out), ptr(z), z.stride(0), B, Rh, Rw, ptr(w10), ptr(dz),
          ptr(partial), ptr(dw10), ptr(db10), dt(z), stream())
     return dz
diff --git a/pcss-unet_amd/nsm_amd/unet.py b/pcss-unet_amd/nsm_amd/unet.py
--- a/pcss-unet_amd/nsm_amd/unet.py
+++ b/pcss-unet_amd/nsm_amd/unet.py
@@ -838,13 +838,20 @@
                     cur = s.Z
                 elif k != 9 and LAZY_DECODER and cdt == torch.bfloat16:
                     cur = ops.Lazy(s.Y2, s.bn2, res)
+                elif k == 9 and training and cdt == torch.float32:
+                    cur = None
                 else:
                     cur = ops.bn_act(s.Y2, s.bn2, SLOPE, res=res,
                                      amax=_x_slot(amax, k + 1) if k < 9 else None)
                 h, w = th, tw
         z9 = cur
         with ops.stage("head.fwd"):
-            out = ops.head_fwd(z9, B, Rh, Rw, mod.conv10.weight.detach(), mod.conv10.bias.detach())
+            if z9 is None:
+                out = ops.head_fwd(saved[9].Y2, B, Rh, Rw, mod.conv10.weight.detach(),
+                                   mod.conv10.bias.detach(), bn=saved[9].bn2, slope=SLOPE)
+            else:
+                out = ops.head_fwd(z9, B, Rh, Rw, mod.conv10.weight.detach(),
+                                   mod.conv10.bias.detach())
 
         if _FROZEN is not None and not training:
             _FROZEN.ready = True
@@ -858,6 +865,7 @@
         ctx.ups = ups
         ctx.meta = (B, C, H, W, orig_hw, Rh, Rw, training)
         ctx.z9 = z9
+        ctx.head_bn = z9 is None
         ctx.save_for_backward(out)
         ctx.params = params
         return out
@@ -906,18 +914,26 @@
         total = flat.numel()
 
         gout = gout.contiguous().to(torch.float32)
+        sb = ctx.saved_blocks
+        gpart = None
         with ops.stage("head.bwd"):
-            G = ops.head_bwd(gout, out, ctx.z9, B, Rh, Rw, mod.conv10.weight.detach(),
-                             grads[mod.conv10.weight], grads[mod.conv10.bias])
-        sb = ctx.saved_blocks
+            if ctx.head_bn:
+                G, gpart = ops.head_bwd(gout, out, None, B, Rh, Rw, mod.conv10.weight.detach(),
+                                        grads[mod.conv10.weight], grads[mod.conv10.bias],
+                                        bnred=_bnred_of(sb[9]), slope=SLOPE)
+            else:
+                G = ops.head_bwd(gout, out, ctx.z9, B, Rh, Rw, mod.conv10.weight.detach(),
+                                 grads[mod.conv10.weight], grads[mod.conv10.bias])
         skip_grad = {}
-        gpart = None
         for k in (9, 8, 7, 6):
             s = sb[k]
             with ops.stage(f"conv{k}.bwd"):
                 dX = _block_bwd(mod.block(k), s, G, grads, True, f"conv{k}", gpart=gpart)
                 h, w, h2, w2, th, tw = ctx.ups[k]
-                if (th, tw) != (h2, w2):
+                if (th, tw) != (h2, w2) and dX.dtype == torch.float32:
+                    dprev, gpart = ops.up2_resize_bwd(dX, B, h, w, th, tw,
+                                                      bnred=_bnred_of(sb[k - 1]))
+                elif (th, tw) != (h2, w2):
                     dprev, gpart = ops.up2_resize_bwd(dX, B, h, w, th, tw), None
                 else:
                     dprev, gpart = ops.resize_bwd(dX, B, h, w, h2, w2, bnred=_bnred_of(sb[k - 1]))
```

After: 697.5 frames/s. 0.893x the previous value.
